# geometryxyz/mental-poker

Measured on AMD Instinct MI355X. Metric: shuffle proofs/sec (prove+verify), higher is better.
Workload: dtype u32 limbs (256-bit Montgomery: 9x29-bit lazy base field, 8x32 scalar field); 1 GPU; pairs: 52-card deck, m=2 n=26, stark curve, shuffle_and_remask + verify_shuffle; rccl_world=1, fixed_base_window_bits=21, unit_counted=prove+verify pairs, streams=1, aggregate_keys=1, transcript_lanes=1, prover_streams=1, pipeline_depth=0, validated_once=False, full=False

## Files before the change

### include/mpshuffle.h

```cpp
#ifndef MPSHUFFLE_H
#define MPSHUFFLE_H

#include <stddef.h>
#include <stdint.h>

#ifdef __cplusplus
extern "C" {
#endif

#define MP_CURVE_STARK 0
#define MP_CURVE_BN254 1
#define MP_CURVE_SECP256K1 2
#define MP_CURVE_BLS12_377 3

#define MP_OK 0
#define MP_ERR_BAD_ENCODING (-1)
#define MP_ERR_BAD_PERMUTATION (-2)
#define MP_ERR_BAD_ARGUMENT (-3)
#define MP_ERR_NO_DEVICE (-4)
#define MP_ERR_INTERNAL (-5)

typedef struct mp_ctx mp_ctx;
typedef struct mp_table mp_table;

int mp_ctx_create(int curve_id, int device, mp_ctx** out);
void mp_ctx_destroy(mp_ctx* ctx);
const char* mp_last_error(void);
const char* mp_check_name(int code);
size_t mp_proof_size(uint32_t m, uint32_t n);
size_t mp_params_size(uint32_t n);
size_t mp_point_size(int curve_id);
size_t mp_proof_size_curve(int curve_id, uint32_t m, uint32_t n);
size_t mp_params_size_curve(int curve_id, uint32_t n);

void* mp_host_alloc(size_t bytes);
void mp_host_free(void* p);
int mp_set_io_chunk(mp_table* t, size_t proofs);

int mp_setup(mp_ctx* ctx, uint32_t m, uint32_t n, const uint8_t seed[32], uint8_t* out_params);

int mp_table_create(mp_ctx* ctx, uint32_t m, uint32_t n, const uint8_t* params, const uint8_t* shared_key,
                    mp_table** out);
int mp_table_create_ex(mp_ctx* ctx, uint32_t m, uint32_t n, const uint8_t* params, const uint8_t* shared_key,
                       uint32_t fb_window_bits, mp_table** out);
uint32_t mp_table_window_bits(const mp_table* t);
void mp_table_destroy(mp_table* t);

int mp_shuffle_and_remask(mp_table* t, const uint8_t* deck, const uint8_t* masking_factors,
                          const uint32_t* permutation, const uint8_t prover_seed[32], uint8_t* out_deck,
                          uint8_t* out_proof);
int mp_verify_shuffle(mp_table* t, const uint8_t* deck, const uint8_t* shuffled_deck, const uint8_t* proof,
                      size_t proof_len);
int mp_shuffle_and_remask_keyed(mp_table* t, const uint8_t* shared_key, const uint8_t* deck, const uint8_t* masking_factors,
                                const uint32_t* permutation, const uint8_t prover_seed[32], uint8_t* out_deck, uint8_t* out_proof);
int mp_verify_shuffle_keyed(mp_table* t, const uint8_t* shared_key, const uint8_t* deck, const uint8_t* shuffled_deck,
                            const uint8_t* proof, size_t proof_len);
int mp_set_coalesce(mp_table* t, size_t max_batch, uint32_t max_wait_us);
int mp_coalesce_stats(const mp_table* t, uint64_t out[8]);

int mp_shuffle_and_remask_batch(mp_table* t, size_t B, const uint8_t* decks, const uint8_t* masking_factors,
                                const uint32_t* permutations, const uint8_t* prover_seeds, uint8_t* out_decks,
                                uint8_t* out_proofs, int32_t* status);
int mp_verify_shuffle_batch(mp_table* t, size_t B, const uint8_t* decks, const uint8_t* shuffled_decks,
                            const uint8_t* proofs, int32_t* status);

int mp_shuffle_and_remask_batch_dev(mp_table* t, size_t B, const void* d_decks, const void* d_masking_factors,
                                    const void* d_permutations, const void* d_prover_seeds, void* d_out_decks,
                                    void* d_out_proofs, void* d_status);
int mp_verify_shuffle_batch_dev(mp_table* t, size_t B, const void* d_decks, const void* d_shuffled_decks,
                                const void* d_proofs, void* d_status);
int mp_table_create_params(mp_ctx* ctx, uint32_t m, uint32_t n, const uint8_t* params, uint32_t fb_window_bits, mp_table** out);
int mp_shuffle_and_remask_batch_keys(mp_table* t, size_t B, const uint8_t* shared_keys, const uint8_t* decks,
                                     const uint8_t* masking_factors, const uint32_t* permutations, const uint8_t* prover_seeds,
                                     uint8_t* out_decks, uint8_t* out_proofs, int32_t* status);
int mp_verify_shuffle_batch_keys(mp_table* t, size_t B, const uint8_t* shared_keys, const uint8_t* decks,
                                 const uint8_t* shuffled_decks, const uint8_t* proofs, int32_t* status);
int mp_shuffle_and_remask_batch_keys_dev(mp_table* t, size_t B, const void* d_keys, const void* d_decks,
                                         const void* d_masking_factors, const void* d_permutations, const void* d_prover_seeds,
                                         void* d_out_decks, void* d_out_proofs, void* d_status);
int mp_verify_shuffle_batch_keys_dev(mp_table* t, size_t B, const void* d_keys, const void* d_decks, const void* d_shuffled_decks,
                                     const void* d_proofs, void* d_status);
typedef struct mp_keyset mp_keyset;
int mp_keyset_create(mp_table* t, size_t n_keys, const uint8_t* keys, mp_keyset** out);
void mp_keyset_destroy(mp_keyset* ks);
size_t mp_keyset_size(const mp_keyset* ks);
int mp_shuffle_and_remask_batch_keyset_dev(mp_table* t, const mp_keyset* ks, size_t B, const void* d_key_index, const void* d_decks,
                                           const void* d_masking_factors, const void* d_permutations, const void* d_prover_seeds,
                                           void* d_out_decks, void* d_out_proofs, void* d_status);
int mp_verify_shuffle_batch_keyset_dev(mp_table* t, const mp_keyset* ks, size_t B, const void* d_key_index, const void* d_decks,
                                       const void* d_shuffled_decks, const void* d_proofs, void* d_status);
int mp_verify_shuffle_chain(mp_table* t, size_t tables, uint32_t links, const uint8_t* shared_keys, const uint8_t* decks,
                            const uint8_t* proofs, int32_t* status);
int mp_verify_shuffle_chain_dev(mp_table* t, size_t tables, uint32_t links, const void* d_keys, const void* d_decks, const void* d_proofs,
                                void* d_status);
int mp_sync(mp_ctx* ctx);
int mp_reserve(mp_table* t, size_t B);
int mp_set_latency_batch(mp_table* t, size_t B);
int mp_set_work_split(mp_table* t, int split);
int mp_set_pipeline(mp_table* t, int depth);
int mp_set_plan_params(mp_table* t, int split, uint32_t fixed_terms, uint32_t var_terms, uint32_t table_group, uint32_t norm_chunk,
                       uint32_t window_lanes);
int mp_set_plan_thresholds(mp_table* t, size_t finest, size_t small, size_t latency, size_t medium, size_t wide);
int mp_set_merged_verify(mp_table* t, int on);
int mp_set_group_verify(mp_table* t, uint32_t points_per_group, size_t min_batch);
uint32_t mp_group_size(const mp_table* t, size_t B);
int mp_set_group_refine(mp_table* t, uint32_t points_per_subgroup, uint32_t min_subgroups);
uint64_t mp_reverified_count(const mp_table* t);
int mp_set_group_adapt(mp_table* t, int on);
int mp_set_bucket_min(mp_table* t, size_t terms);
int mp_set_bucket_bits(mp_table* t, uint32_t bits);
#define MP_VALIDATED_DECKS 1u
#define MP_VALIDATED_SHUFFLED 2u
#define MP_VALIDATED_PROOFS 4u
int mp_set_validated(mp_table* t, uint32_t what);
int mp_deck_validate_dev(mp_table* t, size_t decks, const void* d_wire_decks, void* d_status);
int mp_set_bucket_split(mp_table* t, uint32_t min_bits);
int mp_set_chain_max_links(mp_table* t, uint32_t links);
int mp_set_chain_group(mp_table* t, uint32_t tables_per_equation);
int mp_set_chain_slice(mp_table* t, size_t tables_per_pass);
uint32_t mp_chain_group_size(const mp_table* t, size_t tables, uint32_t links, int keyed);
size_t mp_chain_last_slice(const mp_table* t);
int mp_set_transcript_lanes(mp_table* t, uint32_t lanes);
int mp_set_group_lanes(mp_table* t, uint32_t lanes);
int mp_set_toom_cook(mp_table* t, int on);
int mp_set_subgroup_check(mp_table* t, int on);

int mp_remask_batch(mp_table* t, size_t count, const uint8_t* cards, const uint8_t* masking_factors, uint8_t* out);
int mp_msm(mp_table* t, size_t n_msm, size_t k, const uint8_t* scalars, const uint8_t* points, uint8_t* out);
int mp_commit_batch(mp_table* t, size_t count, size_t len, const uint8_t* values, const uint8_t* r, uint8_t* out);

int mp_sigma_prove_batch(mp_table* t, size_t B, uint32_t nbases, const uint8_t* bases, const uint8_t* publics,
                         const uint8_t* witness, const uint8_t* fs_init, const uint8_t* prover_seeds, uint8_t* out_proofs,
                         int32_t* status);
int mp_sigma_verify_batch(mp_table* t, size_t B, uint32_t nbases, const uint8_t* bases, const uint8_t* publics,
                          const uint8_t* proofs, const uint8_t* fs_init, int32_t* status);
int mp_blake2s(const uint8_t* in, size_t len, uint8_t out[32]);

size_t mp_serialized_point_size(int curve_id);
size_t mp_serialized_deck_size(int curve_id, size_t cards);
size_t mp_serialized_params_size(int curve_id, uint32_t n);
size_t mp_serialized_proof_size(int curve_id, uint32_t m, uint32_t n);
int mp_points_serialize(int curve_id, size_t count, const uint8_t* wire_points, uint8_t* out);
int mp_points_deserialize(int curve_id, size_t count, const uint8_t* data, uint8_t* out_wire_points);
int mp_deck_serialize(int curve_id, size_t cards, const uint8_t* wire_deck, uint8_t* out);
int mp_deck_deserialize(int curve_id, const uint8_t* data, size_t len, size_t max_cards, uint8_t* out_wire_deck, size_t* out_cards);
int mp_params_serialize(int curve_id, uint32_t m, uint32_t n, const uint8_t* raw_params, uint8_t* out);
int mp_params_deserialize(int curve_id, const uint8_t* data, size_t len, size_t max_n, uint32_t* m, uint32_t* n, uint8_t* out_raw_params);
int mp_proof_serialize(int curve_id, uint32_t m, uint32_t n, const uint8_t* proof_wire, uint8_t* out);
int mp_proof_deserialize(int curve_id, uint32_t m, uint32_t n, const uint8_t* data, size_t len, uint8_t* out_proof_wire);
int mp_points_deserialize_dev(mp_ctx* ctx, size_t count, const void* d_data, void* d_out_wire_points, void* d_status);
int mp_deck_deserialize_dev(mp_ctx* ctx, size_t decks, size_t cards, const void* d_data, void* d_out_wire_decks, void* d_status);

int mp_profile_enable(mp_ctx* ctx, int on);
int mp_profile_report(mp_ctx* ctx, char* buf, size_t buf_len);
int mp_work_census(mp_table* t, uint64_t* prove_terms, uint64_t* verify_terms, uint64_t* prove_point_ops,
                   uint64_t* verify_point_ops);

int mp_plan_stats(mp_table* t, uint64_t out[16]);

#ifdef __cplusplus
}
#endif
#endif
```

### mental-poker_amd/_native.py

```python
import ctypes
import os
import subprocess

HERE = os.path.dirname(os.path.abspath(__file__))
LIB_PATH = os.path.join(HERE, "libmpshuffle.so")
ROOT = os.path.dirname(HERE)

CURVE_IDS = {"stark": 0, "bn254": 1, "secp256k1": 2, "bls12_377": 3}
MP_ERR_BAD_ENCODING, MP_ERR_BAD_PERMUTATION, MP_ERR_BAD_ARGUMENT, MP_ERR_NO_DEVICE, MP_ERR_INTERNAL = -1, -2, -3, -4, -5

SYMBOLS = [
    "mp_ctx_create", "mp_ctx_destroy", "mp_last_error", "mp_check_name", "mp_proof_size", "mp_params_size",
    "mp_point_size", "mp_proof_size_curve", "mp_params_size_curve", "mp_set_merged_verify", "mp_set_subgroup_check", "mp_set_bucket_min", "mp_set_bucket_bits", "mp_set_bucket_split", "mp_set_validated", "mp_deck_validate_dev", "mp_set_chain_max_links", "mp_set_chain_group", "mp_set_chain_slice", "mp_chain_group_size", "mp_chain_last_slice", "mp_set_transcript_lanes", "mp_set_group_lanes", "mp_set_work_split", "mp_set_group_verify", "mp_group_size", "mp_set_group_refine", "mp_reverified_count", "mp_set_group_adapt", "mp_set_pipeline", "mp_set_plan_params", "mp_set_plan_thresholds", "mp_set_toom_cook", "mp_host_alloc", "mp_host_free", "mp_set_io_chunk", "mp_shuffle_and_remask_batch_keys", "mp_table_create_params",
    "mp_verify_shuffle_batch_keys", "mp_shuffle_and_remask_batch_keys_dev", "mp_verify_shuffle_batch_keys_dev",
    "mp_keyset_create", "mp_keyset_destroy", "mp_keyset_size", "mp_shuffle_and_remask_batch_keyset_dev", "mp_verify_shuffle_batch_keyset_dev",
    "mp_setup", "mp_table_create", "mp_table_create_ex", "mp_table_window_bits", "mp_table_destroy", "mp_shuffle_and_remask", "mp_verify_shuffle",
    "mp_shuffle_and_remask_keyed", "mp_verify_shuffle_keyed", "mp_set_coalesce", "mp_coalesce_stats",
    "mp_shuffle_and_remask_batch", "mp_verify_shuffle_batch", "mp_shuffle_and_remask_batch_dev",
    "mp_verify_shuffle_batch_dev", "mp_verify_shuffle_chain", "mp_verify_shuffle_chain_dev", "mp_sync", "mp_reserve", "mp_set_latency_batch", "mp_remask_batch", "mp_msm", "mp_commit_batch",
    "mp_profile_enable", "mp_profile_report", "mp_work_census", "mp_plan_stats", "mp_sigma_prove_batch",
    "mp_sigma_verify_batch", "mp_blake2s",
    "mp_serialized_point_size", "mp_serialized_deck_size", "mp_serialized_params_size", "mp_serialized_proof_size",
    "mp_points_serialize", "mp_points_deserialize", "mp_deck_serialize", "mp_deck_deserialize", "mp_params_serialize",
    "mp_params_deserialize", "mp_proof_serialize", "mp_proof_deserialize", "mp_points_deserialize_dev", "mp_deck_deserialize_dev",
]


class NativeError(RuntimeError):
    def __init__(self, code, text):
        super().__init__("mpshuffle error %d: %s" % (code, text))
        self.code = code


class NoDeviceError(NativeError):
    pass


SOURCES = ["capi.hip"] + [f % c for c in ("stark", "bn254", "secp256k1", "bls12_377") for f in ("curve_%s.hip", "curve_%s_msm.hip")]


def build(verbose=False):
    from concurrent.futures import ThreadPoolExecutor
    csrc = os.path.join(HERE, "csrc")
    objdir = os.path.join(csrc, "_obj")
    os.makedirs(objdir, exist_ok=True)
    headers = [os.path.join(csrc, f) for f in os.listdir(csrc) if f.endswith(".hpp")]
    headers.append(os.path.join(ROOT, "include", "mpshuffle.h"))
    hdr_time = max(os.path.getmtime(h) for h in headers)
    hipcc = os.environ.get("HIPCC", "/opt/rocm/bin/hipcc")
    flags = ["--offload-arch=gfx950", "-O3", "-std=c++17", "-fPIC", "-mllvm", "-amdgpu-sched-strategy=max-ilp",
             "-mllvm", "-pragma-unroll-threshold=1000000"]

    def compile_one(src):
        obj = os.path.join(objdir, src.replace(".hip", ".o"))
        spath = os.path.join(csrc, src)
        if os.path.exists(obj) and os.path.getmtime(obj) >= max(hdr_time, os.path.getmtime(spath)):
            return obj, False
        cmd = [hipcc] + flags + ["-c", spath, "-o", obj]
        if verbose:
            print(" ".join(cmd), flush=True)
        subprocess.check_call(cmd)
        return obj, True

    def compile_check():
        src = os.path.join(ROOT, "tools", "quadcheck", "quad_check.hip")
        exe = os.path.join(ROOT, "tools", "quadcheck", "quad_check")
        if not os.path.exists(src) or (os.path.exists(exe) and os.path.getmtime(exe) >= max(hdr_time, os.path.getmtime(src))):
            return
        cmd = [hipcc] + [f for f in flags if f != "-fPIC"] + ["-I", csrc, src, "-o", exe]
        if verbose:
            print(" ".join(cmd), flush=True)
        try:
            subprocess.check_call(cmd)
        except (subprocess.CalledProcessError, OSError) as e:
            print("warning: tools/quadcheck/quad_check did not build (%s); the library is unaffected" % e, flush=True)

    with ThreadPoolExecutor(max_workers=len(SOURCES) + 1) as ex:
        chk = ex.submit(compile_check)
        res = list(ex.map(compile_one, SOURCES))
        chk.result()
    objs = [r[0] for r in res]
    if any(r[1] for r in res) or not os.path.exists(LIB_PATH) or os.path.getmtime(LIB_PATH) < max(os.path.getmtime(o) for o in objs):
        cmd = [hipcc, "--offload-arch=gfx950", "-shared", "-fPIC", "-pthread", "-o", LIB_PATH] + objs
        if verbose:
            print(" ".join(cmd), flush=True)
        subprocess.check_call(cmd)
    mc = os.path.join(HERE, "mad_counts.json")
    gen = os.path.join(ROOT, "tools", "gen_mad_counts.py")
    if os.path.exists(gen) and (not os.path.exists(mc) or os.path.getmtime(mc) < max(hdr_time, os.path.getmtime(gen))):
        import importlib.util
        spec = importlib.util.spec_from_file_location("gen_mad_counts", gen)
        mod = importlib.util.module_from_spec(spec)
        spec.loader.exec_module(mod)
        mod.main([f for f in flags if f != "-fPIC"])
    return LIB_PATH


def bind(cdll):
    c = ctypes
    u8p, u32p, i32p = c.c_void_p, c.c_void_p, c.c_void_p
    cdll.mp_ctx_create.argtypes = [c.c_int, c.c_int, c.POINTER(c.c_void_p)]
    cdll.mp_ctx_destroy.argtypes = [c.c_void_p]
    cdll.mp_ctx_destroy.restype = None
    cdll.mp_last_error.restype = c.c_char_p
    cdll.mp_check_name.argtypes = [c.c_int]
    cdll.mp_check_name.restype = c.c_char_p
    cdll.mp_proof_size.argtypes = [c.c_uint32, c.c_uint32]
    cdll.mp_proof_size.restype = c.c_size_t
    cdll.mp_params_size.argtypes = [c.c_uint32]
    cdll.mp_params_size.restype = c.c_size_t
    cdll.mp_set_merged_verify.argtypes = [c.c_void_p, c.c_int]
    cdll.mp_set_subgroup_check.argtypes = [c.c_void_p, c.c_int]
    cdll.mp_set_bucket_min.argtypes = [c.c_void_p, c.c_size_t]
    cdll.mp_set_bucket_bits.argtypes = [c.c_void_p, c.c_uint32]
    cdll.mp_set_bucket_split.argtypes = [c.c_void_p, c.c_uint32]
    cdll.mp_set_validated.argtypes = [c.c_void_p, c.c_uint32]
    cdll.mp_deck_validate_dev.argtypes = [c.c_void_p, c.c_size_t, c.c_void_p, c.c_void_p]
    cdll.mp_set_toom_cook.argtypes = [c.c_void_p, c.c_int]
    cdll.mp_set_chain_max_links.argtypes = [c.c_void_p, c.c_uint32]
    cdll.mp_set_chain_group.argtypes = [c.c_void_p, c.c_uint32]
    cdll.mp_set_chain_slice.argtypes = [c.c_void_p, c.c_size_t]
    cdll.mp_chain_group_size.argtypes = [c.c_void_p, c.c_size_t, c.c_uint32, c.c_int]
    cdll.mp_chain_group_size.restype = c.c_uint32
    cdll.mp_chain_last_slice.argtypes = [c.c_void_p]
    cdll.mp_chain_last_slice.restype = c.c_size_t
    cdll.mp_set_transcript_lanes.argtypes = [c.c_void_p, c.c_uint32]
    cdll.mp_set_group_lanes.argtypes = [c.c_void_p, c.c_uint32]
    cdll.mp_set_work_split.argtypes = [c.c_void_p, c.c_int]
    cdll.mp_set_group_verify.argtypes = [c.c_void_p, c.c_uint32, c.c_size_t]
    cdll.mp_group_size.argtypes = [c.c_void_p, c.c_size_t]
    cdll.mp_group_size.restype = c.c_uint32
    cdll.mp_set_group_refine.argtypes = [c.c_void_p, c.c_uint32, c.c_uint32]
    cdll.mp_reverified_count.argtypes = [c.c_void_p]
    cdll.mp_set_group_adapt.argtypes = [c.c_void_p, c.c_int]
    cdll.mp_reverified_count.restype = c.c_uint64
    cdll.mp_set_pipeline.argtypes = [c.c_void_p, c.c_int]
    cdll.mp_set_plan_params.argtypes = [c.c_void_p, c.c_int] + [c.c_uint32] * 5
    cdll.mp_set_plan_thresholds.argtypes = [c.c_void_p] + [c.c_size_t] * 5
    cdll.mp_set_io_chunk.argtypes = [c.c_void_p, c.c_size_t]
    cdll.mp_host_alloc.argtypes = [c.c_size_t]
    cdll.mp_host_alloc.restype = c.c_void_p
    cdll.mp_host_free.argtypes = [c.c_void_p]
    cdll.mp_host_free.restype = None
    cdll.mp_point_size.argtypes = [c.c_int]
    cdll.mp_point_size.restype = c.c_size_t
    cdll.mp_proof_size_curve.argtypes = [c.c_int, c.c_uint32, c.c_uint32]
    cdll.mp_proof_size_curve.restype = c.c_size_t
    cdll.mp_params_size_curve.argtypes = [c.c_int, c.c_uint32]
    cdll.mp_params_size_curve.restype = c.c_size_t
    cdll.mp_setup.argtypes = [c.c_void_p, c.c_uint32, c.c_uint32, u8p, u8p]
    cdll.mp_table_create.argtypes = [c.c_void_p, c.c_uint32, c.c_uint32, u8p, u8p, c.POINTER(c.c_void_p)]
    cdll.mp_table_create_ex.argtypes = [c.c_void_p, c.c_uint32, c.c_uint32, u8p, u8p, c.c_uint32, c.POINTER(c.c_void_p)]
    cdll.mp_table_window_bits.argtypes = [c.c_void_p]
    cdll.mp_table_window_bits.restype = c.c_uint32
    cdll.mp_table_destroy.argtypes = [c.c_void_p]
    cdll.mp_table_destroy.restype = None
    cdll.mp_shuffle_and_remask.argtypes = [c.c_void_p, u8p, u8p, u32p, u8p, u8p, u8p]
    cdll.mp_verify_shuffle.argtypes = [c.c_void_p, u8p, u8p, u8p, c.c_size_t]
    cdll.mp_shuffle_and_remask_keyed.argtypes = [c.c_void_p, u8p, u8p, u8p, u32p, u8p, u8p, u8p]
    cdll.mp_verify_shuffle_keyed.argtypes = [c.c_void_p, u8p, u8p, u8p, u8p, c.c_size_t]
    cdll.mp_set_coalesce.argtypes = [c.c_void_p, c.c_size_t, c.c_uint32]
    cdll.mp_coalesce_stats.argtypes = [c.c_void_p, c.POINTER(c.c_uint64)]
    cdll.mp_shuffle_and_remask_batch.argtypes = [c.c_void_p, c.c_size_t, u8p, u8p, u32p, u8p, u8p, u8p, i32p]
    cdll.mp_verify_shuffle_batch.argtypes = [c.c_void_p, c.c_size_t, u8p, u8p, u8p, i32p]
    cdll.mp_shuffle_and_remask_batch_dev.argtypes = [c.c_void_p, c.c_size_t] + [c.c_void_p] * 7
    cdll.mp_verify_shuffle_batch_dev.argtypes = [c.c_void_p, c.c_size_t] + [c.c_void_p] * 4
    cdll.mp_table_create_params.argtypes = [c.c_void_p, c.c_uint32, c.c_uint32, u8p, c.c_uint32, c.POINTER(c.c_void_p)]
    cdll.mp_shuffle_and_remask_batch_keys.argtypes = [c.c_void_p, c.c_size_t, u8p, u8p, u8p, u32p, u8p, u8p, u8p, i32p]
    cdll.mp_verify_shuffle_batch_keys.argtypes = [c.c_void_p, c.c_size_t, u8p, u8p, u8p, u8p, i32p]
    cdll.mp_shuffle_and_remask_batch_keys_dev.argtypes = [c.c_void_p, c.c_size_t] + [c.c_void_p] * 8
    cdll.mp_verify_shuffle_batch_keys_dev.argtypes = [c.c_void_p, c.c_size_t] + [c.c_void_p] * 5
    cdll.mp_keyset_create.argtypes = [c.c_void_p, c.c_size_t, u8p, c.POINTER(c.c_void_p)]
    cdll.mp_keyset_destroy.argtypes = [c.c_void_p]
    cdll.mp_keyset_destroy.restype = None
    cdll.mp_keyset_size.argtypes = [c.c_void_p]
    cdll.mp_keyset_size.restype = c.c_size_t
    cdll.mp_shuffle_and_remask_batch_keyset_dev.argtypes = [c.c_void_p, c.c_void_p, c.c_size_t] + [c.c_void_p] * 8
    cdll.mp_verify_shuffle_batch_keyset_dev.argtypes = [c.c_void_p, c.c_void_p, c.c_size_t] + [c.c_void_p] * 5
    cdll.mp_verify_shuffle_chain.argtypes = [c.c_void_p, c.c_size_t, c.c_uint32, u8p, u8p, u8p, i32p]
    cdll.mp_verify_shuffle_chain_dev.argtypes = [c.c_void_p, c.c_size_t, c.c_uint32] + [c.c_void_p] * 4
    cdll.mp_sync.argtypes = [c.c_void_p]
    cdll.mp_reserve.argtypes = [c.c_void_p, c.c_size_t]
    cdll.mp_set_latency_batch.argtypes = [c.c_void_p, c.c_size_t]
    cdll.mp_remask_batch.argtypes = [c.c_void_p, c.c_size_t, u8p, u8p, u8p]
    cdll.mp_msm.argtypes = [c.c_void_p, c.c_size_t, c.c_size_t, u8p, u8p, u8p]
    cdll.mp_commit_batch.argtypes = [c.c_void_p, c.c_size_t, c.c_size_t, u8p, u8p, u8p]
    cdll.mp_profile_enable.argtypes = [c.c_void_p, c.c_int]
    cdll.mp_profile_report.argtypes = [c.c_void_p, c.c_char_p, c.c_size_t]
    cdll.mp_work_census.argtypes = [c.c_void_p] + [c.POINTER(c.c_uint64)] * 4
    cdll.mp_plan_stats.argtypes = [c.c_void_p, c.POINTER(c.c_uint64)]
    cdll.mp_sigma_prove_batch.argtypes = [c.c_void_p, c.c_size_t, c.c_uint32, u8p, u8p, u8p, u8p, u8p, u8p, i32p]
    cdll.mp_sigma_verify_batch.argtypes = [c.c_void_p, c.c_size_t, c.c_uint32, u8p, u8p, u8p, u8p, i32p]
    cdll.mp_blake2s.argtypes = [u8p, c.c_size_t, u8p]
    for fn, at in (("mp_serialized_point_size", [c.c_int]), ("mp_serialized_deck_size", [c.c_int, c.c_size_t]),
                   ("mp_serialized_params_size", [c.c_int, c.c_uint32]), ("mp_serialized_proof_size", [c.c_int, c.c_uint32, c.c_uint32])):
        getattr(cdll, fn).argtypes = at
        getattr(cdll, fn).restype = c.c_size_t
    cdll.mp_points_serialize.argtypes = [c.c_int, c.c_size_t, u8p, u8p]
    cdll.mp_points_deserialize.argtypes = [c.c_int, c.c_size_t, u8p, u8p]
    cdll.mp_deck_serialize.argtypes = [c.c_int, c.c_size_t, u8p, u8p]
    cdll.mp_deck_deserialize.argtypes = [c.c_int, u8p, c.c_size_t, c.c_size_t, u8p, c.POINTER(c.c_size_t)]
    cdll.mp_params_serialize.argtypes = [c.c_int, c.c_uint32, c.c_uint32, u8p, u8p]
    cdll.mp_params_deserialize.argtypes = [c.c_int, u8p, c.c_size_t, c.c_size_t, c.POINTER(c.c_uint32), c.POINTER(c.c_uint32), u8p]
    cdll.mp_points_deserialize_dev.argtypes = [c.c_void_p, c.c_size_t, c.c_void_p, c.c_void_p, c.c_void_p]
    cdll.mp_deck_deserialize_dev.argtypes = [c.c_void_p, c.c_size_t, c.c_size_t, c.c_void_p, c.c_void_p, c.c_void_p]
    cdll.mp_proof_serialize.argtypes = [c.c_int, c.c_uint32, c.c_uint32, u8p, u8p]
    cdll.mp_proof_deserialize.argtypes = [c.c_int, c.c_uint32, c.c_uint32, u8p, c.c_size_t, u8p]
    return cdll


_LIB = None


def load():
    global _LIB
    if _LIB is None:
        if not os.path.exists(LIB_PATH):
            raise ImportError("libmpshuffle.so is not built (run `python -c 'import __graft_entry__ as g; g.build()'`); "
# ... 31 lines not shown

    def points_deserialize(self, data):
        k = len(data) // self.cb
        if k * self.cb != len(data):
            raise NativeError(MP_ERR_BAD_ENCODING, "whole compressed points expected")
        out = (ctypes.c_uint8 * max(k * self.pb, 1))()
        self._chk(self.lib.mp_points_deserialize(self.cid, k, _in(data), out))
        return bytes(out)[:k * self.pb]

    def deck_serialize(self, wire):
        k = len(wire) // (2 * self.pb)
        if 2 * k * self.pb != len(wire):
            raise NativeError(MP_ERR_BAD_ARGUMENT, "whole cards expected")
        out = (ctypes.c_uint8 * self.lib.mp_serialized_deck_size(self.cid, k))()
        self._chk(self.lib.mp_deck_serialize(self.cid, k, _in(wire), out))
        return bytes(out)

    def deck_deserialize(self, data):
        cap = max(len(data) // (2 * self.cb), 1)
        out = (ctypes.c_uint8 * (cap * 2 * self.pb))()
        k = ctypes.c_size_t()
        self._chk(self.lib.mp_deck_deserialize(self.cid, _in(data), len(data), cap, out, ctypes.byref(k)))
        return bytes(out)[:k.value * 2 * self.pb]

    def params_serialize(self, m, n, raw):
        if len(raw) != self.pb * (n + 3):
            raise NativeError(MP_ERR_BAD_ARGUMENT, "parameters: wrong length")
        out = (ctypes.c_uint8 * self.lib.mp_serialized_params_size(self.cid, n))()
        self._chk(self.lib.mp_params_serialize(self.cid, m, n, _in(raw), out))
        return bytes(out)

    def params_deserialize(self, data):
        cap = max(len(data) // self.cb, 1)
        out = (ctypes.c_uint8 * (self.pb * (cap + 3)))()
        m, n = ctypes.c_uint32(), ctypes.c_uint32()
        self._chk(self.lib.mp_params_deserialize(self.cid, _in(data), len(data), cap, ctypes.byref(m), ctypes.byref(n), out))
        return m.value, n.value, bytes(out)[:self.pb * (n.value + 3)]

    def proof_serialize(self, m, n, wire):
        if len(wire) != self.lib.mp_proof_size_curve(self.cid, m, n):
            raise NativeError(MP_ERR_BAD_ARGUMENT, "proof: wrong length")
        out = (ctypes.c_uint8 * self.proof_serialized_size(m, n))()
        self._chk(self.lib.mp_proof_serialize(self.cid, m, n, _in(wire), out))
        return bytes(out)

    def proof_deserialize(self, m, n, data):
        out = (ctypes.c_uint8 * self.lib.mp_proof_size_curve(self.cid, m, n))()
        self._chk(self.lib.mp_proof_deserialize(self.cid, m, n, _in(data), len(data), out))
        return bytes(out)


class Engine:

    def __init__(self, curve="stark", device=0, lib=None):
        self.lib = lib if lib is not None else load()
        self.curve = curve
        h = ctypes.c_void_p()
        rc = self.lib.mp_ctx_create(CURVE_IDS[curve], device, ctypes.byref(h))
        if rc != 0:
            text = self.lib.mp_last_error().decode()
            raise (NoDeviceError if rc == MP_ERR_NO_DEVICE else NativeError)(rc, text)
        self.h = h
        self.point_bytes = self.lib.mp_point_size(CURVE_IDS[curve])

    def close(self):
        if getattr(self, "h", None):
            self.lib.mp_ctx_destroy(self.h)
            self.h = None

    def __del__(self):
        try:
            self.close()
        except Exception:
            pass

    def _chk(self, rc):
        if rc < 0:
            raise NativeError(rc, self.lib.mp_last_error().decode())
        return rc

    def check_name(self, code):
        return self.lib.mp_check_name(code).decode()

    def proof_size(self, m, n):
        return self.lib.mp_proof_size_curve(CURVE_IDS[self.curve], m, n)

    def blake2s(self, data):
        out = (ctypes.c_uint8 * 32)()
        self._chk(self.lib.mp_blake2s(_in(data), len(data), out))
        return bytes(out)

    def setup(self, m, n, seed):
        out = (ctypes.c_uint8 * self.lib.mp_params_size_curve(CURVE_IDS[self.curve], n))()
        self._chk(self.lib.mp_setup(self.h, m, n, _in(seed), out))
        return bytes(out)

    def table(self, m, n, params, shared_key, fb_bits=8):
        return Table(self, m, n, params, shared_key, fb_bits)

    def sync(self):
        self._chk(self.lib.mp_sync(self.h))

    def points_deserialize_dev(self, count, d_data, d_out_wire, d_status):
        self._chk(self.lib.mp_points_deserialize_dev(self.h, count, d_data, d_out_wire, d_status))

    def deck_deserialize_dev(self, decks, cards, d_data, d_out_wire_decks, d_status):
        self._chk(self.lib.mp_deck_deserialize_dev(self.h, decks, cards, d_data, d_out_wire_decks, d_status))

    def profile_enable(self, on=True):
        self._chk(self.lib.mp_profile_enable(self.h, 1 if on else 0))

    def profile_report(self):
        buf = ctypes.create_string_buffer(1 << 16)
        self._chk(self.lib.mp_profile_report(self.h, buf, len(buf)))
        out = {}
        self.last_profile_items = {}
        for line in buf.value.decode().splitlines():
            f = line.split()
            out[f[0]] = (int(f[1]), float(f[2]))
            if len(f) > 3:
                self.last_profile_items[f[0]] = int(f[3])
        return out


class KeySet:

    def __init__(self, table, keys):
        self.table, self.lib = table, table.lib
        if len(keys) == 0 or len(keys) % table.pb:
            raise ValueError("keys: expected a whole number of %d-byte points" % table.pb)
        self.size = len(keys) // table.pb
        h = ctypes.c_void_p()
        table.eng._chk(self.lib.mp_keyset_create(table.h, self.size, _in(keys), ctypes.byref(h)))
        self.h = h

    def close(self):
        if getattr(self, "h", None):
            self.lib.mp_keyset_destroy(self.h)
            self.h = None

    def __del__(self):
        try:
            self.close()
        except Exception:
            pass


class Table:

    def __init__(self, eng, m, n, params, shared_key, fb_bits=8):
        self.eng, self.lib, self.m, self.n, self.N = eng, eng.lib, m, n, m * n
        self.fb_bits = fb_bits
        self.params, self.shared_key = bytes(params), (bytes(shared_key) if shared_key is not None else None)
        self.pb = eng.point_bytes
        self.cb = 2 * eng.point_bytes
        if len(self.params) != self.pb * (n + 3) or (self.shared_key is not None and len(self.shared_key) != self.pb):
            raise NativeError(MP_ERR_BAD_ARGUMENT, "parameters / shared key have the wrong length")
        h = ctypes.c_void_p()
        if self.shared_key is None:
            eng._chk(self.lib.mp_table_create_params(eng.h, m, n, _in(self.params), fb_bits, ctypes.byref(h)))
        else:
            eng._chk(self.lib.mp_table_create_ex(eng.h, m, n, _in(self.params), _in(self.shared_key), fb_bits, ctypes.byref(h)))
        self.h = h
        self.fb_bits = self.lib.mp_table_window_bits(h)
        self.proof_bytes = eng.proof_size(m, n)

# ... 277 lines not shown
```

### mental-poker_amd/csrc/capi.hip

```cpp
#include <algorithm>
#include <cstring>

#include "engine_base.hpp"
#include "coalesce.hpp"

namespace mp {
std::string& last_error() {
  static thread_local std::string e;
  return e;
}
static inline size_t proof_size_bytes_(uint32_t m, uint32_t n) { return proof_size_bytes(m, n); }
}

using namespace mp;

#define MP_ENTER(CTX)                                          \
  std::lock_guard<std::recursive_mutex> mp_lock_((CTX)->mu);   \
  rt::set_device((CTX)->device)
#define MP_TRY try {
#define MP_CATCH                                                                     \
  }                                                                                  \
  catch (const std::invalid_argument& e) { return fail(MP_ERR_BAD_ENCODING, e.what()); } \
  catch (const std::exception& e) { return fail(MP_ERR_INTERNAL, e.what()); }

// ... 11 lines not shown
    case 0: return ser_scalars_ok_Stark(count, in);
    case 1: return ser_scalars_ok_Bn254(count, in);
    case 3: return ser_scalars_ok_Bls12_377(count, in);
    default: return ser_scalars_ok_Secp256k1(count, in);
  }
}
const int kCurveBits[4] = {252, 254, 256, 377};
struct Group {
  bool point;
  uint32_t count;
  bool vec;
  uint32_t vec_len;
};
std::vector<Group> proof_schema(uint32_t m, uint32_t n) {
  return {
      {true, m, true, m}, {true, m, true, m}, {true, 1, false, 0}, {true, m, true, m},
      {true, 1, false, 0}, {true, 1, false, 0}, {true, 2 * m + 1, true, 2 * m + 1},
      {false, n, true, n}, {false, n, true, n}, {false, 1, false, 0}, {false, 1, false, 0}, {false, 1, false, 0},
      {true, 1, false, 0}, {true, 1, false, 0}, {true, 1, false, 0},
      {false, n, true, n}, {false, n, true, n}, {false, 1, false, 0}, {false, 1, false, 0},
      {true, 1, false, 0}, {true, 2 * m, true, 2 * m}, {true, 4 * m, true, 2 * m},
      {false, n, true, n}, {false, 1, false, 0}, {false, 1, false, 0}, {false, 1, false, 0}, {false, 1, false, 0}};
}
void put_u64(uint8_t* p, uint64_t v) { memcpy(p, &v, 8); }
uint64_t get_u64(const uint8_t* p) {
  uint64_t v;
  memcpy(&v, p, 8);
  return v;
}
bool curve_ok(int c) { return c >= 0 && c <= 3; }
struct NoPipeline {
  mp_table* t;
  int keep;
  explicit NoPipeline(mp_table* tt) : t(tt), keep(tt->pipeline) {
    if (keep) t->flush();
    t->pipeline = 0;
  }
  ~NoPipeline() { t->pipeline = keep; }
};
}

extern "C" {

const char* mp_last_error(void) { return mp::last_error().c_str(); }
const char* mp_check_name(int code) {
  switch (code) {
    case 0: return "Ok";
    case 1: return "Hadamard Product (5.1)";
    case 2: return "Zero Argument (5.2)";
    case 3: return "Single Value Product (5.3)";
    case 4: return "Multi-Exponentiation Argument (4)";
    case 5: return "Schnorr Identification";
    case 6: return "Chaum-Pedersen";
    case MP_ERR_BAD_ENCODING: return "IoError: bad encoding";
    case MP_ERR_BAD_PERMUTATION: return "IoError: not a permutation";
    case MP_ERR_BAD_ARGUMENT: return "IoError: bad argument";
    case MP_ERR_NO_DEVICE: return "IoError: no MI355X device";
    default: return "IoError: internal";
  }
}
size_t mp_proof_size(uint32_t m, uint32_t n) { return proof_size_bytes(m, n); }
size_t mp_params_size(uint32_t n) { return (size_t)(n + 3) * 64; }
size_t mp_point_size(int curve_id) { return curve_id == MP_CURVE_BLS12_377 ? 96 : 64; }
size_t mp_proof_size_curve(int curve_id, uint32_t m, uint32_t n) { return proof_size_bytes(m, n, (uint32_t)mp_point_size(curve_id)); }
size_t mp_params_size_curve(int curve_id, uint32_t n) { return (size_t)(n + 3) * mp_point_size(curve_id); }

int mp_ctx_create(int curve_id, int device, mp_ctx** out) {
  if (!out) return fail(MP_ERR_BAD_ARGUMENT, "null out pointer");
  if (curve_id < 0 || curve_id > 3) return fail(MP_ERR_BAD_ARGUMENT, "unknown curve id");
  MP_TRY
  int ndev = rt::device_count();
  if (ndev <= 0 || device < 0 || device >= ndev)
    return fail(MP_ERR_NO_DEVICE, "no HIP device: libmpshuffle has no CPU path (runtime " MP_RT_NAME ")");
  rt::set_device(device);
  mp_ctx* c = new mp_ctx();
  c->curve = curve_id;
  c->device = device;
  c->stream = rt::stream_create();
  c->vstream = rt::stream_create();
  c->side = rt::stream_create();
  c->vside = rt::stream_create();
  c->h2d = c->vstream;
  c->d2h = c->vside;
  c->ev_fork = rt::event_create();
  c->ev_shuf = rt::event_create();
  c->ev_tab = rt::event_create();
  c->ev_vfork = rt::event_create();
  c->ev_vshuf = rt::event_create();
  c->ev_vtab = rt::event_create();
  c->ev_vin = rt::event_create();
  *out = c;
  return MP_OK;
  MP_CATCH
}
static void ctx_release(mp_ctx* ctx) {
  for (rt::Stream st : {ctx->stream, ctx->side, ctx->vstream, ctx->vside})
    if (st) rt::stream_destroy(st);
  for (rt::Event e : {ctx->ev_fork, ctx->ev_shuf, ctx->ev_tab, ctx->ev_vfork, ctx->ev_vshuf, ctx->ev_vtab, ctx->ev_vin})
    if (e) rt::event_destroy(e);
  delete ctx;
}
void mp_ctx_destroy(mp_ctx* ctx) {
  if (!ctx) return;
  {
    std::lock_guard<std::recursive_mutex> lock(ctx->mu);
    if (!ctx->tables.empty()) {
      ctx->dying = true;
      return;
    }
  }
  ctx_release(ctx);
}
int mp_setup(mp_ctx* ctx, uint32_t m, uint32_t n, const uint8_t seed[32], uint8_t* out_params) {
  if (!ctx || !seed || !out_params || m < 2 || n < 2) return fail(MP_ERR_BAD_ARGUMENT, "mp_setup: bad argument");
  MP_TRY
  MP_ENTER(ctx);
  switch (ctx->curve) {
    case 0: return setup_Stark(ctx, m, n, seed, out_params);
    case 1: return setup_Bn254(ctx, m, n, seed, out_params);
    case 3: return setup_Bls12_377(ctx, m, n, seed, out_params);
    default: return setup_Secp256k1(ctx, m, n, seed, out_params);
  }
  MP_CATCH
}

static uint32_t auto_window_bits(int curve, uint32_t n) {
  size_t free_b = 0, total_b = 0;
  rt::mem_info(&free_b, &total_b);
  const uint32_t sbits[4] = {252, 254, 256, 253};
  const size_t pbytes = curve == MP_CURVE_BLS12_377 ? 96 : 64;
  for (uint32_t bits : {21u, 20u, 16u}) {
    if (bits == 21 && sbits[curve] > 252) continue;
    const double tbl = (double)(n + 5) * ((sbits[curve] + bits - 1) / bits) * (double)((1u << bits) - 1u) * (double)pbytes;
    if (tbl <= 0.30 * (double)free_b && 3.3 * tbl <= 0.85 * (double)free_b) return bits;
  }
  return 8;
}
int mp_table_create(mp_ctx* ctx, uint32_t m, uint32_t n, const uint8_t* params, const uint8_t* shared_key, mp_table** out) {
  return mp_table_create_ex(ctx, m, n, params, shared_key, 0, out);
}
int mp_table_create_ex(mp_ctx* ctx, uint32_t m, uint32_t n, const uint8_t* params, const uint8_t* shared_key,
                       uint32_t fb_window_bits, mp_table** out) {
  if (!ctx || !params || !shared_key || !out) return fail(MP_ERR_BAD_ARGUMENT, "mp_table_create: null pointer");
  if (m < 2 || n < 2 || (uint64_t)m * n > 4096) return fail(MP_ERR_BAD_ARGUMENT, "mp_table_create: need m >= 2, n >= 2, m*n <= 4096");
  MP_TRY
  MP_ENTER(ctx);
  const bool auto_bits = fb_window_bits == 0;
  if (auto_bits) fb_window_bits = auto_window_bits(ctx->curve, n);
  int rc = MP_OK;
  mp_table* t = nullptr;
  auto make = [&](uint32_t bits) {
    switch (ctx->curve) {
      case 0: return make_table_Stark(ctx, m, n, params, shared_key, bits, &rc);
      case 1: return make_table_Bn254(ctx, m, n, params, shared_key, bits, &rc);
      case 3: return make_table_Bls12_377(ctx, m, n, params, shared_key, bits, &rc);
      default: return make_table_Secp256k1(ctx, m, n, params, shared_key, bits, &rc);
    }
  };
  if (!auto_bits) {
    t = make(fb_window_bits);
  } else {
    for (;;) {
      try {
        t = make(fb_window_bits);
        break;
      } catch (const std::exception& e) {
// ... 1 lines not shown
        if (fb_window_bits <= 8 || (!strstr(e.what(), "hipMalloc") && !strstr(e.what(), "memory"))) throw;
        fb_window_bits = fb_window_bits > 20 ? 20 : (fb_window_bits > 16 ? 16 : 8);
      }
    }
  }
  if (rc != MP_OK) {
    delete t;
    return rc;
  }
  t->co = new mp_coalescer();
  ctx->tables.push_back(t);
  *out = t;
  return MP_OK;
  MP_CATCH
}
int mp_table_create_params(mp_ctx* ctx, uint32_t m, uint32_t n, const uint8_t* params, uint32_t fb_window_bits, mp_table** out) {
  int rc = mp_table_create_ex(ctx, m, n, params, params, fb_window_bits, out);
  if (rc == MP_OK) (*out)->keyless = true;
  return rc;
}
void mp_table_destroy(mp_table* t) {
  if (!t) return;
  try {
    MP_ENTER(t->ctx);
    t->flush();
  } catch (...) {
  }
  mp_ctx* ctx = t->ctx;
  bool last = false;
  {
    std::lock_guard<std::recursive_mutex> lock(ctx->mu);
    auto& reg = ctx->tables;
    reg.erase(std::remove(reg.begin(), reg.end(), t), reg.end());
    for (auto& st : t->io) {
      if (st.up) rt::event_destroy(st.up);
      if (st.done) rt::event_destroy(st.done);
      if (st.down) rt::event_destroy(st.down);
    }
    delete t->co;
    delete t;
    last = ctx->dying && reg.empty();
  }
  if (last) ctx_release(ctx);
}
void* mp_host_alloc(size_t bytes) {
  try {
    return rt::host_alloc(bytes);
  } catch (const std::exception& e) {
    fail(MP_ERR_INTERNAL, e.what());
    return nullptr;
  }
}
void mp_host_free(void* p) { rt::host_free(p); }

uint32_t mp_table_window_bits(const mp_table* t) {
  if (!t) return 0;
  std::lock_guard<std::recursive_mutex> mp_lock_(t->ctx->mu);
  return t->fb_bits;
}
int mp_set_latency_batch(mp_table* t, size_t B) {
  if (!t) return fail(MP_ERR_BAD_ARGUMENT, "mp_set_latency_batch: null table");
  std::lock_guard<std::recursive_mutex> mp_lock_(t->ctx->mu);
  t->set_latency_batch(B);
  return MP_OK;
}
int mp_set_io_chunk(mp_table* t, size_t proofs) {
  if (!t) return fail(MP_ERR_BAD_ARGUMENT, "mp_set_io_chunk: null table");
  std::lock_guard<std::recursive_mutex> mp_lock_(t->ctx->mu);
  t->io_chunk = proofs;
  return MP_OK;
}
int mp_set_merged_verify(mp_table* t, int on) {
  if (!t) return fail(MP_ERR_BAD_ARGUMENT, "mp_set_merged_verify: null table");
  std::lock_guard<std::recursive_mutex> mp_lock_(t->ctx->mu);
  t->set_merged_verify(on != 0);
  return MP_OK;
}
int mp_set_group_refine(mp_table* t, uint32_t points_per_subgroup, uint32_t min_subgroups) {
  if (!t) return fail(MP_ERR_BAD_ARGUMENT, "mp_set_group_refine: null table");
  if (points_per_subgroup > BUCKET_TERMS_MAX - 4096) return fail(MP_ERR_BAD_ARGUMENT, "mp_set_group_refine: at most 585 728 points per equation");
  std::lock_guard<std::recursive_mutex> mp_lock_(t->ctx->mu);
  t->set_group_refine(points_per_subgroup, min_subgroups);
  return MP_OK;
}
uint64_t mp_reverified_count(const mp_table* t) {
  if (!t) return 0;
  std::lock_guard<std::recursive_mutex> mp_lock_(t->ctx->mu);
  return t->reverified();
}
int mp_set_group_adapt(mp_table* t, int on) {
  if (!t) return fail(MP_ERR_BAD_ARGUMENT, "mp_set_group_adapt: null table");
  std::lock_guard<std::recursive_mutex> mp_lock_(t->ctx->mu);
  t->set_group_adapt(on != 0);
  return MP_OK;
}
int mp_set_bucket_min(mp_table* t, size_t terms) {
  if (!t) return fail(MP_ERR_BAD_ARGUMENT, "mp_set_bucket_min: null table");
  MP_TRY
  MP_ENTER(t->ctx);
  t->set_bucket_min((uint32_t)std::min<size_t>(terms, 0x7FFFFFFFu));
  return MP_OK;
  MP_CATCH
}
int mp_set_bucket_bits(mp_table* t, uint32_t bits) {
  if (!t) return fail(MP_ERR_BAD_ARGUMENT, "mp_set_bucket_bits: null table");
  if (bits != 0 && (bits < 8 || bits > 14)) return fail(MP_ERR_BAD_ARGUMENT, "mp_set_bucket_bits: 0 (by size) or 8 .. 14");
  MP_TRY
  MP_ENTER(t->ctx);
  t->set_bucket_bits(bits);
  return MP_OK;
  MP_CATCH
}
int mp_set_bucket_split(mp_table* t, uint32_t min_bits) {
  if (!t) return fail(MP_ERR_BAD_ARGUMENT, "mp_set_bucket_split: null table");
  if (min_bits < 10 || min_bits > 15) return fail(MP_ERR_BAD_ARGUMENT, "mp_set_bucket_split: 10 .. 15 (none)");
  MP_TRY
  MP_ENTER(t->ctx);
  t->flush();
  t->bucket_split_bits = min_bits;
  return MP_OK;
  MP_CATCH
}
int mp_set_validated(mp_table* t, uint32_t what) {
  if (!t) return fail(MP_ERR_BAD_ARGUMENT, "mp_set_validated: null table");
  if (what & ~(MP_VALIDATED_DECKS | MP_VALIDATED_SHUFFLED | MP_VALIDATED_PROOFS)) return fail(MP_ERR_BAD_ARGUMENT, "mp_set_validated: unknown flag");
  MP_TRY
  MP_ENTER(t->ctx);
  t->flush();
  t->validated = what;
  return MP_OK;
  MP_CATCH
}
int mp_deck_validate_dev(mp_table* t, size_t decks, const void* d_wire_decks, void* d_status) {
  if (!t || !decks || !d_wire_decks || !d_status || decks >= ((size_t)1 << 31)) return fail(MP_ERR_BAD_ARGUMENT, "mp_deck_validate_dev: bad argument");
  MP_TRY
  MP_ENTER(t->ctx);
  t->validate_decks_dev(decks, (const uint8_t*)d_wire_decks, (int32_t*)d_status);
  return MP_OK;
  MP_CATCH
}
int mp_set_chain_max_links(mp_table* t, uint32_t links) {
  if (!t) return fail(MP_ERR_BAD_ARGUMENT, "mp_set_chain_max_links: null table");
  std::lock_guard<std::recursive_mutex> mp_lock_(t->ctx->mu);
  t->chain_max_links = links;
  return MP_OK;
}
int mp_set_chain_slice(mp_table* t, size_t tables_per_pass) {
  if (!t) return fail(MP_ERR_BAD_ARGUMENT, "mp_set_chain_slice: null table");
  std::lock_guard<std::recursive_mutex> mp_lock_(t->ctx->mu);
  t->chain_slice = tables_per_pass;
  return MP_OK;
}
int mp_set_chain_group(mp_table* t, uint32_t tables_per_equation) {
  if (!t) return fail(MP_ERR_BAD_ARGUMENT, "mp_set_chain_group: null table");
  if (tables_per_equation > 4094) return fail(MP_ERR_BAD_ARGUMENT, "mp_set_chain_group: at most 4 094 tables per equation");
  std::lock_guard<std::recursive_mutex> mp_lock_(t->ctx->mu);
  t->chain_group = tables_per_equation;
  return MP_OK;
}
int mp_set_transcript_lanes(mp_table* t, uint32_t lanes) {
  if (!t) return fail(MP_ERR_BAD_ARGUMENT, "mp_set_transcript_lanes: null table");
  if (lanes != 0 && lanes != 1 && lanes != 4) return fail(MP_ERR_BAD_ARGUMENT, "mp_set_transcript_lanes: 0 (by batch size), 1 or 4");
  std::lock_guard<std::recursive_mutex> mp_lock_(t->ctx->mu);
  t->fs_lanes = lanes;
  return MP_OK;
}
// ... 795 lines not shown
```

### mental-poker_amd/csrc/curve.hpp

```cpp
#pragma once
#include "field.hpp"

namespace mp {

template <class C>
struct Aff {
  Fe<typename C::FqP> x, y;
};
template <class C>
struct Jac {
  Fe<typename C::FqP> X, Y, Z;
};

template <class C>
struct Cofactor {
  static constexpr bool ONE = C::ID != 3;
  static constexpr uint32_t H[4] = {0x00000000u, 0x00000000u, 0x30000000u, 0x170b5d44u};
};

template <class C>
MP_HD bool aff_is_inf(const Aff<C>& a) {
  return fe_is_zero(a.x) && fe_is_zero(a.y);
}
template <class C>
// ... 78 lines not shown
  if (aff_is_inf<C>(q)) return;
  if (fe_is_zero(p.Z)) {
    p.X = q.x;
    p.Y = q.y;
    p.Z = fe_one<F>();
    return;
  }
  const Fe<F> Z1Z1 = fe_sqr<F>(p.Z);
  const Fe<F> U2 = fe_mul<F>(q.x, Z1Z1);
  const Fe<F> S2 = fe_mul<F>(fe_mul<F>(q.y, p.Z), Z1Z1);
  const Fe<F> H = fe_sub<F>(U2, p.X);
  const Fe<F> Rr = fe_sub<F>(S2, p.Y);
  if (fe_is_zero(H)) {
    if (fe_is_zero(Rr))
      jac_dbl_ip<C>(p);
    else
      p.Z = fe_zero<F>();
    return;
  }
  const Fe<F> HH = fe_sqr<F>(H);
  const Fe<F> HHH = fe_mul<F>(H, HH);
  const Fe<F> V = fe_mul<F>(p.X, HH);
  const Fe<F> X3 = fe_sub<F>(fe_sub<F>(fe_sqr<F>(Rr), HHH), fe_dbl<F>(V));
  p.Y = fe_sub<F>(fe_mul<F>(Rr, fe_sub<F>(V, X3)), fe_mul<F>(p.Y, HHH));
  p.Z = fe_mul<F>(p.Z, H);
  p.X = X3;
}
template <class C>
MP_HD Jac<C> jac_madd(const Jac<C>& p, const Aff<C>& q) {
  Jac<C> r = p;
  jac_madd_ip<C>(r, q);
  return r;
}

template <class C>
MP_HD void jac_add_ip(Jac<C>& p, const Jac<C>& q) {
  typedef typename C::FqP F;
  if (fe_is_zero(q.Z)) return;
  if (fe_is_zero(p.Z)) {
    p = q;
    return;
  }
  const Fe<F> Z1Z1 = fe_sqr<F>(p.Z), Z2Z2 = fe_sqr<F>(q.Z);
  const Fe<F> U1 = fe_mul<F>(p.X, Z2Z2), U2 = fe_mul<F>(q.X, Z1Z1);
  const Fe<F> S1 = fe_mul<F>(fe_mul<F>(p.Y, q.Z), Z2Z2), S2 = fe_mul<F>(fe_mul<F>(q.Y, p.Z), Z1Z1);
  const Fe<F> H = fe_sub<F>(U2, U1);
  const Fe<F> Rr = fe_sub<F>(S2, S1);
  if (fe_is_zero(H)) {
    if (fe_is_zero(Rr))
      jac_dbl_ip<C>(p);
    else
      p.Z = fe_zero<F>();
    return;
  }
  const Fe<F> HH = fe_sqr<F>(H);
  const Fe<F> HHH = fe_mul<F>(H, HH);
  const Fe<F> V = fe_mul<F>(U1, HH);
  const Fe<F> X3 = fe_sub<F>(fe_sub<F>(fe_sqr<F>(Rr), HHH), fe_dbl<F>(V));
  p.Y = fe_sub<F>(fe_mul<F>(Rr, fe_sub<F>(V, X3)), fe_mul<F>(S1, HHH));
  p.Z = fe_mul<F>(fe_mul<F>(p.Z, q.Z), H);
  p.X = X3;
}
template <class C>
MP_HD Jac<C> jac_add(const Jac<C>& p, const Jac<C>& q) {
  Jac<C> r = p;
  jac_add_ip<C>(r, q);
  return r;
}

template <class C>
struct Xyzz {
  Fe<typename C::FqP> X, Y, ZZ, ZZZ;
};
template <class C>
MP_HD Xyzz<C> xyzz_inf() {
  Xyzz<C> p;
  p.X = fe_one<typename C::FqP>();
  p.Y = fe_one<typename C::FqP>();
  p.ZZ = fe_zero<typename C::FqP>();
  p.ZZZ = fe_zero<typename C::FqP>();
  return p;
}
template <class C>
MP_HD void xyzz_dbl_ip(Xyzz<C>& p) {
  typedef typename C::FqP F;
  if (fe_is_zero(p.ZZ)) return;
  if (fe_is_zero(p.Y)) {
    p.ZZ = fe_zero<F>();
    p.ZZZ = fe_zero<F>();
    return;
  }
  const Fe<F> U = fe_dbl<F>(p.Y);
  const Fe<F> V = fe_sqr<F>(U);
  const Fe<F> W = fe_mul<F>(U, V);
  const Fe<F> S = fe_mul<F>(p.X, V);
  const Fe<F> XX = fe_sqr<F>(p.X);
  const Fe<F> M = C::A == 1 ? fe_triple_add<F>(XX, fe_sqr<F>(p.ZZ)) : fe_add<F>(fe_dbl<F>(XX), XX);
  const Fe<F> X3 = fe_sub_dbl<F>(fe_sqr<F>(M), S);
  p.Y = fe_mulsub<F>(M, fe_sub_lazy<F>(S, X3), W, p.Y);
  p.X = X3;
  p.ZZ = fe_mul<F>(V, p.ZZ);
  p.ZZZ = fe_mul<F>(W, p.ZZZ);
}
template <class C, bool PROBE = false>
MP_HD void xyzz_madd_signed_ip(Xyzz<C>& p, const Aff<C>& q, bool neg) {
  typedef typename C::FqP F;
  if (aff_is_inf<C>(q)) return;
  if (fe_is_zero(p.ZZ)) {
    p.X = q.x;
    p.Y = neg ? fe_neg<F>(q.y) : q.y;
    p.ZZ = fe_one<F>();
    p.ZZZ = fe_one<F>();
    return;
  }
  Fe<F> qy = q.y;
  if constexpr (LazySub<F>::ON) {
    const Fe<F> ny = fe_neg_lazy<F>(q.y);
#pragma unroll
    for (int i = 0; i < 9; ++i) qy.v[i] = neg ? ny.v[i] : q.y.v[i];
  } else {
    if (neg) qy = fe_neg<F>(q.y);
  }
  const Fe<F> Pd = fe_sub_wide<F>(fe_mul<F>(q.x, p.ZZ), p.X);
  const Fe<F> Rr = fe_sub_wide<F>(fe_mul<F>(qy, p.ZZZ), p.Y);
  if (fe_is_zero(Pd)) {
    if (!PROBE && fe_is_zero(Rr)) {
      xyzz_dbl_ip<C>(p);
    } else {
      p.ZZ = fe_zero<F>();
      p.ZZZ = fe_zero<F>();
    }
    return;
  }
  const Fe<F> PP = fe_sqr<F>(Pd);
  const Fe<F> PPP = fe_mul<F>(Pd, PP);
  const Fe<F> Q = fe_mul<F>(p.X, PP);
  const Fe<F> X3 = fe_sub_sub_dbl<F>(fe_sqr<F>(Rr), PPP, Q);
  p.Y = fe_mulsub<F>(Rr, fe_sub_lazy<F>(Q, X3), p.Y, PPP);
  p.X = X3;
  p.ZZ = fe_mul<F>(p.ZZ, PP);
  p.ZZZ = fe_mul<F>(p.ZZZ, PPP);
}
template <class C, bool PROBE = false>
MP_HD void xyzz_madd_ip(Xyzz<C>& p, const Aff<C>& q) {
  xyzz_madd_signed_ip<C, PROBE>(p, q, false);
}
template <class C, bool PROBE = false>
MP_HD void xyzz_add_ip(Xyzz<C>& p, const Xyzz<C>& q) {
  typedef typename C::FqP F;
  if (fe_is_zero(q.ZZ)) return;
  if (fe_is_zero(p.ZZ)) {
    p = q;
    return;
  }
  const Fe<F> U1 = fe_mul<F>(p.X, q.ZZ), U2 = fe_mul<F>(q.X, p.ZZ);
  const Fe<F> S1 = fe_mul<F>(p.Y, q.ZZZ), S2 = fe_mul<F>(q.Y, p.ZZZ);
  const Fe<F> Pd = fe_sub<F>(U2, U1);
  const Fe<F> Rr = fe_sub<F>(S2, S1);
  if (fe_is_zero(Pd)) {
    if (!PROBE && fe_is_zero(Rr)) {
      xyzz_dbl_ip<C>(p);
    } else {
      p.ZZ = fe_zero<F>();
      p.ZZZ = fe_zero<F>();
    }
    return;
  }
  const Fe<F> PP = fe_sqr<F>(Pd);
  const Fe<F> PPP = fe_mul<F>(Pd, PP);
  const Fe<F> Q = fe_mul<F>(U1, PP);
  const Fe<F> X3 = fe_sub_sub_dbl<F>(fe_sqr<F>(Rr), PPP, Q);
  p.Y = fe_mulsub<F>(Rr, fe_sub_lazy<F>(Q, X3), S1, PPP);
  p.X = X3;
  p.ZZ = fe_mul<F>(fe_mul<F>(p.ZZ, q.ZZ), PP);
  p.ZZZ = fe_mul<F>(fe_mul<F>(p.ZZZ, q.ZZZ), PPP);
}
template <class C>
MP_HD Jac<C> xyzz_to_jac(const Xyzz<C>& p) {
  typedef typename C::FqP F;
  Jac<C> j;
  if (fe_is_zero(p.ZZ)) return jac_inf<C>();
  j.X = fe_mul<F>(p.X, p.ZZ);
  j.Y = fe_mul<F>(p.Y, p.ZZZ);
  j.Z = p.ZZ;
  return j;
}

template <class C>
MP_HD Aff<C> jac_to_aff_with_zinv(const Jac<C>& j, const Fe<typename C::FqP>& zinv) {
  typedef typename C::FqP F;
  Fe<F> zi2 = fe_sqr<F>(zinv);
  Aff<C> a;
  a.x = fe_mul<F>(j.X, zi2);
  a.y = fe_mul<F>(fe_mul<F>(j.Y, zi2), zinv);
  return a;
}

}
```

### mental-poker_amd/csrc/engine_base.hpp

```cpp
#pragma once
#include <algorithm>
#include <cstring>
#include <deque>
#include <map>
#include <memory>
#include <sstream>
#include <string>
#include <mutex>
#include <vector>

#include "../../include/mpshuffle.h"
#include "hash.hpp"
#include "layout.hpp"

namespace mp {

std::string& last_error();
inline int fail(int code, const std::string& msg) {
  last_error() = msg;
  return code;
}

template <class T>
struct DevBuf {
// ... 10 lines not shown
    p = (T*)rt::dmalloc(count * sizeof(T));
    n = count;
    if (zero) rt::dzero(p, count * sizeof(T), s);
  }
  void upload(const std::vector<T>& v, rt::Stream s) {
    alloc(v.size() ? v.size() : 1, s, false);
    if (!v.empty()) rt::h2d(p, v.data(), v.size() * sizeof(T), s);
  }
};

struct Profiler {
  bool on = false;
  struct Rec {
    const char* name;
    rt::Event a, b;
    uint64_t items;
  };
  std::vector<Rec> recs;
  std::vector<rt::Event> pool;
  rt::Event get() {
    if (!pool.empty()) {
      rt::Event e = pool.back();
      pool.pop_back();
      return e;
    }
    return rt::event_create();
  }
  void begin(const char* name, rt::Stream s, uint64_t items = 0) {
    if (!on) return;
    Rec r{name, get(), get(), items};
    rt::event_record(r.a, s);
    recs.push_back(r);
  }
  void end(rt::Stream s) {
    if (!on) return;
    rt::event_record(recs.back().b, s);
  }
  std::string report() {
    std::map<std::string, std::pair<long, double>> acc;
    std::map<std::string, uint64_t> items;
    std::vector<std::string> order;
    for (auto& r : recs) {
      float ms = rt::event_ms(r.a, r.b);
      if (!acc.count(r.name)) order.push_back(r.name);
      acc[r.name].first += 1;
      acc[r.name].second += ms;
      items[r.name] += r.items;
      pool.push_back(r.a);
      pool.push_back(r.b);
    }
    recs.clear();
    std::ostringstream os;
    for (auto& k : order) os << k << " " << acc[k].first << " " << acc[k].second << " " << items[k] << "\n";
    return os.str();
  }
  ~Profiler() {
    for (auto& r : recs) {
      rt::event_destroy(r.a);
      rt::event_destroy(r.b);
    }
    for (auto e : pool) rt::event_destroy(e);
  }
};

}

struct mp_ctx {
  std::recursive_mutex mu;
  int curve = 0;
  int device = 0;
  mp::rt::Stream stream{};
  mp::rt::Stream h2d{}, d2h{};
  mp::rt::Stream side{};
  mp::rt::Event ev_fork{}, ev_shuf{}, ev_tab{};
  mp::rt::Stream vstream{}, vside{};
  mp::rt::Event ev_vfork{}, ev_vshuf{}, ev_vtab{}, ev_vin{};
  std::vector<mp_table*> tables;
  bool dying = false;
  mp::DevBuf<uint32_t> sq_ghalf, sq_hh, sq_rr, sq_chain;
  uint32_t sq_geom[4] = {0, 0, 0, 0};
  uint32_t sq_exp[12] = {0};
  mp::Profiler prof;
  uint32_t bk_slots = 0;
};
namespace mp {
struct LaneSwap {
  mp_ctx* c;
  explicit LaneSwap(mp_ctx* ctx) : c(ctx) { swap(); }
  ~LaneSwap() { swap(); }
  LaneSwap(const LaneSwap&) = delete;
  LaneSwap& operator=(const LaneSwap&) = delete;
  void swap() {
    std::swap(c->stream, c->vstream);
    std::swap(c->side, c->vside);
    std::swap(c->ev_fork, c->ev_vfork);
    std::swap(c->ev_shuf, c->ev_vshuf);
    std::swap(c->ev_tab, c->ev_vtab);
  }
};
}

static const uint32_t FSQ_MAX_BATCH = 32768;
static const uint32_t PROVE_INIT_WAVE_MAX = 32768;
static const uint32_t OVERLAP_MAX_BATCH = 32768;
static const uint32_t SCAL3D_SPLIT_MAX_BATCH = 4096;
#define MP_WAVE_RUN(NAME, C, nwaves, lds_words, args)                             \
  do {                                                                            \
    ctx->prof.begin(#NAME, ctx->stream, (uint64_t)(nwaves));                      \
    MP_WAVE_LAUNCH(NAME, C, ctx->stream, (nwaves), (lds_words), (args));          \
    ctx->prof.end(ctx->stream);                                                   \
  } while (0)
#define MP_RUN(NAME, C, nx, ny, args)                      \
  do {                                                     \
    ctx->prof.begin(#NAME, ctx->stream, (uint64_t)(nx) * (ny)); \
    MP_LAUNCH(NAME, C, ctx->stream, (nx), (ny), (args));   \
    ctx->prof.end(ctx->stream);                            \
  } while (0)

struct mp_io_stage {
  mp::DevBuf<uint8_t> in0, in1, in2, in3, out0, out1, keys;
  mp::DevBuf<uint32_t> perm;
  mp::DevBuf<int32_t> status;
  mp::rt::Event up = nullptr, done = nullptr, down = nullptr;
  bool used = false;
};
struct mp_keyset {
  mp_table* owner = nullptr;
  size_t K = 0;
  mp::DevBuf<uint32_t> wire;
  mp::DevBuf<uint32_t> FB;
  uint32_t bits = 0, windows = 0, entries = 0;
};
struct mp_coalescer;
struct mp_table {
  mp_ctx* ctx = nullptr;
  mp_coalescer* co = nullptr;
  mp_io_stage io[2];
  size_t io_chunk = 0;
  uint32_t m = 0, n = 0, N = 0;
  uint32_t point_bytes = 64;
  uint32_t fb_bits = 8;
  bool keyless = false;
  uint32_t bucket_bits = 0;
  uint32_t validated = 0;
  uint32_t bucket_split_bits = 12;
  uint32_t chain_max_links = 0;
  size_t chain_slice = 0;
  uint32_t chain_group = 0;
  uint32_t fs_lanes = 0;
  uint32_t group_lanes = 0;
  int forced_split = -1;
  int pipeline = 0;
  virtual ~mp_table() {}
  virtual void flush() = 0;
  virtual void reserve(size_t B) = 0;
  virtual void set_latency_batch(size_t B) = 0;
  virtual void set_merged_verify(bool on) = 0;
  virtual void set_subgroup_check(bool on) = 0;
  virtual void set_bucket_min(uint32_t terms) = 0;
  virtual void set_bucket_bits(uint32_t bits) = 0;
  virtual void set_toom_cook(bool on) = 0;
  virtual void set_group_verify(uint32_t links, size_t min_batch) = 0;
  virtual uint32_t group_size_of(size_t B) const = 0;
  virtual void set_group_refine(uint32_t points, uint32_t min_groups) = 0;
  virtual void set_group_adapt(bool on) = 0;
  virtual uint64_t reverified() const = 0;
  virtual int set_plan_params(int plan, uint32_t fch, uint32_t vch, uint32_t grp, uint32_t nch, uint32_t vsp) = 0;
  virtual void set_plan_thresholds(size_t tiny, size_t small, size_t latency, size_t medium, size_t wide) = 0;
  virtual void prove_dev(size_t B, const uint8_t* decks, const uint8_t* rho, const uint32_t* perm, const uint8_t* seeds,
                         uint8_t* out_decks, uint8_t* out_proofs, int32_t* status, const uint8_t* keys = nullptr,
                         const mp_keyset* ks = nullptr, const uint32_t* kidx = nullptr) = 0;
  virtual void verify_dev(size_t B, const uint8_t* decks, const uint8_t* shuf, const uint8_t* proofs, int32_t* status,
                          const uint8_t* keys = nullptr, const mp_keyset* ks = nullptr, const uint32_t* kidx = nullptr) = 0;
  virtual int keyset_build(mp_keyset& ks, size_t K, const uint8_t* keys_host) = 0;
  virtual void verify_chain_dev(size_t T, uint32_t L, const uint8_t* decks, const uint8_t* proofs, int32_t* status,
                                const uint8_t* keys = nullptr) = 0;
  virtual size_t chain_lane_bytes(uint32_t L, bool keyed) = 0;
  virtual size_t chain_lanes_held() const = 0;
  virtual void validate_decks_dev(size_t count, const uint8_t* decks, int32_t* status) = 0;
  virtual uint32_t chain_group_size(size_t T, uint32_t L, bool keyed) const = 0;
  size_t chain_last_slice = 0;
  virtual void remask_host(size_t count, const uint8_t* cards, const uint8_t* rho, uint8_t* out) = 0;
  virtual void msm_host(size_t n_msm, size_t k, const uint8_t* scalars, const uint8_t* points, uint8_t* out) = 0;
  virtual void commit_host(size_t count, size_t len, const uint8_t* values, const uint8_t* r, uint8_t* out) = 0;
  virtual void sigma_host(bool prove, size_t B, uint32_t nb, const uint8_t* bases, const uint8_t* publics, const uint8_t* witness,
                          const uint8_t* fs_init, const uint8_t* seeds, uint8_t* proofs, int32_t* status) = 0;
  virtual void census(uint64_t* pt, uint64_t* vt, uint64_t* po, uint64_t* vo) = 0;
  virtual void plan_stats(uint64_t out[16]) = 0;
};


namespace mp {
#define MP_DECLARE_CURVE(NAME)                                                                                          \
  mp_table* make_table_##NAME(mp_ctx* ctx, uint32_t m, uint32_t n, const uint8_t* params, const uint8_t* pk,           \
                              uint32_t fb_bits, int* rc);                                                              \
  int setup_##NAME(mp_ctx* ctx, uint32_t m, uint32_t n, const uint8_t seed[32], uint8_t* out);                                   \
  long ser_points_##NAME(bool de, size_t count, const uint8_t* in, uint8_t* out);                                                \
  int decompress_dev_##NAME(mp_ctx* ctx, size_t groups, uint32_t per_group, uint32_t prefix, const uint8_t* d_in, uint8_t* d_out, \
                            int32_t* d_status);                                                                                   \
// ... 7 lines not shown
```

### mental-poker_amd/csrc/engine_core.hpp

```cpp
#pragma once
#include "engine_base.hpp"
#include "kernels_bucket.hpp"
#include "kernels_decompress.hpp"
#include "kernels_sigma.hpp"
#include "serialize_host.hpp"
#include "setup_host.hpp"

namespace mp {

static const uint32_t FCHUNK = 8;
static const uint32_t VCHUNK = 64;
static const uint32_t NORM_CHUNK = 64;
static const uint32_t BUCKET_MIN = 2048;
static const uint32_t BUCKET_MIN_SMALL_BATCH = 512;

struct PhaseDev {
  DevBuf<Term> recode, tables, fterms, vterms, cterms, cterms2, cterms0;
  DevBuf<Job> fjobs, vjobs, cjobs, cjobs2, cjobs0;
  DevBuf<BJob> bjobs;
  DevBuf<Term> bterms;
  DevBuf<BTermPos> bpos;
  DevBuf<Job> wcjobs;
  DevBuf<Term> wcterms;
  DevBuf<BJob> wjobs;
// ... 597 lines not shown
    if ((uint64_t)count * ph.n_bterms >= ((uint64_t)1 << 32) || (uint64_t)count * ph.n_b * bw + 8ull * bucket_slots() >= ((uint64_t)1 << 32)) throw std::runtime_error(too_large);
    BRecodeArgs ra{S, D, ph.bterms.p, ph.bpos.p, sstride, bw, ph.n_bterms, dstride, c};
    MP_RUN(k_bucket_recode, C, count * ph.n_bterms, 1, ra);
    if (c >= bucket_split_bits) {
      const uint32_t NBK = bk_buckets(c), XW = XyzzWords<C>::N, gmax = bk_chunks(ph.b_kpad_max), units = bk_units(c);
      if (gmax > BK_CHUNKS_MAX) throw std::runtime_error("bucket method: more than 589 824 terms in one multi-scalar multiplication with windows of 12 bits or more");
      const size_t per_item = ((size_t)ph.b_kpad_max + (size_t)NBK * XW) * 4 + (size_t)gmax * bk_offs_row(c) * 2, per_eq = per_item * ph.n_b * bw;
      if (!bk_pass_eqs || bk_pass_bytes != per_eq) {
        size_t free_b = 0, total_b = 0;
        rt::mem_info(&free_b, &total_b);
        const size_t have = (w.bk_sorted.n + w.bk_park.n) * 4 + w.bk_offs.n * 2;
        const size_t budget = total_b ? std::min<size_t>((size_t)12 << 30, (free_b + have) / 4) : (size_t)1 << 30;
        bk_pass_eqs = (uint32_t)std::max<size_t>(1, std::min<size_t>(budget / per_eq, 0x7FFFFFFFu));
        bk_pass_bytes = per_eq;
      }
      const uint32_t pass = std::min(count, std::max(bk_pass_eqs, 1u));
      const size_t items_max = (size_t)pass * ph.n_b * bw;
      if (items_max * units >= ((uint64_t)1 << 32)) throw std::runtime_error(too_large);
      w.bk_sorted.alloc(items_max * ph.b_kpad_max, s, false);
      w.bk_offs.alloc(items_max * gmax * bk_offs_row(c), s, false);
      w.bk_park.alloc(items_max * NBK * XW, s, false);
      w.bk_quarters.alloc(items_max * 8 * XW, s, false);
      for (uint32_t e0 = 0; e0 < count; e0 += pass) {
        const uint32_t ne = std::min(pass, count - e0), items = ne * ph.n_b * bw;
        const uint32_t acc_lds = bk_acc_lds_words(c, gmax, XW, G_::PW), wpb = rt::waves_per_block(acc_lds), wgs = (items * units + wpb - 1) / wpb;
        BSplitArgs sa{D, w.P.p, w.J.p, ph.bjobs.p, ph.bterms.p, w.Bpad, bw, ph.n_b, dstride, link_stride, c, e0, ne, tile, tile_K,
                      w.bk_sorted.p, w.bk_offs.p, w.bk_park.p, ph.b_kpad_max, gmax, units, wpb, wgs, w.bk_quarters.p};
        ctx->prof.begin("k_bucket_sort", s, (uint64_t)items * gmax);
        MP_BLOCK_LAUNCH(k_bucket_sort, C, s, items * gmax, bk_sort_lds_words(c), sa);
        ctx->prof.end(s);
        MP_WAVE_RUN(k_bucket_acc, C, (wgs + 7u) / 8u * 8u * wpb, acc_lds, sa);
        MP_WAVE_RUN(k_bucket_list, C, (wgs + 7u) / 8u * 8u * wpb, acc_lds, sa);
        MP_WAVE_RUN(k_bucket_reduce, C, items * 4u, 64u * XW, sa);
        MP_RUN(k_bucket_final, C, items, 1, sa);
      }
      BFoldArgs fa{w.J.p, ph.bjobs.p, w.Bpad, bw, 0u, c};
      if (quad_ops(count, ph.n_b)) {
        BFoldQuadArgs qa{fa, count, ph.n_b};
        MP_WAVE_RUN(k_bucket_fold_q, C, quad_waves(count, ph.n_b), 0, qa);
      } else {
        MP_RUN(k_bucket_fold, C, count, ph.n_b, fa);
      }
      return;
    }
    const uint32_t nitems = count * ph.n_b * bw, nslots = std::min(nitems, bucket_slots());
    w.ensure_bucket(bucket_slots(), ph.b_kpad_max, c, XyzzWords<C>::N, s);
    rt::dzero(w.bk_counter.p, 8 * 4, s);
    BucketArgs ba{D, w.P.p, w.J.p, ph.bjobs.p, ph.bterms.p, w.Bpad, bw, ph.n_b, dstride, link_stride, c, nitems, nslots, w.bk_counter.p,
                  count, bk_xcd_affine && count >= 8u ? 8u : 1u, tile, tile_K, bk_stage ? 1u : 0u,
                  w.bk_sorted.p, w.bk_park.p, ph.b_kpad_max, nullptr};
#ifdef MP_EXP_BK_TIMING
    w.bk_timing.alloc((size_t)bucket_slots() * 8, s);
    ba.timing = w.bk_timing.p;
#endif
    ctx->prof.begin("k_bucket_msm", s, nitems);
    MP_WAVE_LAUNCH(k_bucket_msm, C, s, nslots, bk_lds_words(c, XyzzWords<C>::N), ba);
    ctx->prof.end(s);
#ifdef MP_EXP_BK_TIMING
    {
      std::vector<unsigned long long> tm((size_t)nslots * 4);
      rt::d2h(tm.data(), w.bk_timing.p, tm.size() * 8, s);
      rt::stream_sync(s);
      double sum[4] = {0, 0, 0, 0};
      for (size_t i = 0; i < tm.size(); ++i) sum[i & 3] += (double)tm[i];
      fprintf(stderr, "k_bucket_msm items %u slots %u bits %u kpad %u: cycles/wave sort %.0f ranks %.0f additions %.0f reduction %.0f\n", nitems, nslots, c,
              ph.b_kpad_max, sum[0] / nslots, sum[1] / nslots, sum[2] / nslots, sum[3] / nslots);
    }
#endif
    BFoldArgs fa{w.J.p, ph.bjobs.p, w.Bpad, bw, 0u, c};
    if (quad_ops(count, ph.n_b)) {
      BFoldQuadArgs qa{fa, count, ph.n_b};
      MP_WAVE_RUN(k_bucket_fold_q, C, quad_waves(count, ph.n_b), 0, qa);
    } else {
      MP_RUN(k_bucket_fold, C, count, ph.n_b, fa);
    }
  }
  void run_msms(PhaseDev& ph, Workspace& w, uint32_t B) {
    if (ph.n_f) {
      FixedArgs a{w.S.p, w.J.p, FB.p, ph.fjobs.p, ph.fterms.p, w.Bpad, fbg, w.Bpad};
      if (quad_ops(B, ph.n_f)) {
        FixedQuadArgs qa{a, B, ph.n_f};
        MP_WAVE_RUN(k_fixed_msm_q, C, quad_waves(B, ph.n_f), 0, qa);
      } else {
        MP_RUN(k_fixed_msm, C, B, ph.n_f, a);
      }
    }
    if (ph.n_v) {
      VarArgs a{w.D.p, w.T.p, w.J.p, ph.vjobs.p, ph.vterms.p, w.Bpad, nwin, ph.vsplit};
      const uint32_t nvl = ph.n_v * ph.vsplit;
#ifdef MP_EXP_VAR_LDS
      ctx->prof.begin("k_var_msm", ctx->stream);
      hipLaunchKernelGGL((k_var_msm<C>), dim3((B + 255u) / 256u, nvl), dim3(256), MP_EXP_VAR_LDS, ctx->stream, a, (uint32_t)B);
      ctx->prof.end(ctx->stream);
#else
      if (quad_ops(B, nvl)) {
        VarQuadArgs qa{a, B, nvl};
        MP_WAVE_RUN(k_var_msm_q, C, quad_waves(B, nvl), 0, qa);
      } else {
        MP_RUN(k_var_msm, C, B, nvl, a);
      }
#endif
      if (ph.n_wc) {
        CombineArgs ca{w.J.p, w.P.p, ph.wcjobs.p, ph.wcterms.p, w.Bpad};
        run_combine(ca, B, ph.n_wc);
      }
      if (ph.n_w) {
        BFoldArgs fa{w.J.p, ph.wjobs.p, w.Bpad, 0u, nwin, 0u};
        if (quad_ops(B, ph.n_w)) {
          BFoldQuadArgs qa{fa, B, ph.n_w};
          ctx->prof.begin("k_wfold_q", ctx->stream);
          MP_WAVE_LAUNCH(k_bucket_fold_q, C, ctx->stream, quad_waves(B, ph.n_w), 0, qa);
          ctx->prof.end(ctx->stream);
        } else {
          ctx->prof.begin("k_wfold", ctx->stream);
          MP_LAUNCH(k_bucket_fold, C, ctx->stream, B, ph.n_w, fa);
          ctx->prof.end(ctx->stream);
        }
      }
    }
    if (ph.n_b) run_bucket(w, ph, w.S.p, w.Bpad, w.D16.p, (size_t)w.d8_bytes, B, 0u, "bucket recode: batch too large for one launch");
    if (ph.n_c0) {
      CombineArgs a{w.J.p, w.P.p, ph.cjobs0.p, ph.cterms0.p, w.Bpad};
      run_combine(a, B, ph.n_c0);
    }
    if (ph.n_c) {
      CombineArgs a{w.J.p, w.P.p, ph.cjobs.p, ph.cterms.p, w.Bpad};
      run_combine(a, B, ph.n_c);
    }
    if (ph.n_c2) {
      CombineArgs a{w.J.p, w.P.p, ph.cjobs2.p, ph.cterms2.p, w.Bpad};
      run_combine(a, B, ph.n_c2);
    }
  }
  void run_normalize(PhaseDev& ph, Workspace& w, uint32_t B, uint32_t norm_only, uint32_t norm_skip, uint32_t* scratch) {
    std::vector<std::pair<uint32_t, uint32_t>> ranges;
    for (auto& r : ph.normalize)
      if ((norm_only == NO_SLOT || r.first == norm_only) && r.first != norm_skip) ranges.push_back(r);
    for (size_t i = 0; i < ranges.size();) {
      const size_t nr = std::min<size_t>(NORM_MAX_RANGES, ranges.size() - i);
      size_t last_elem = 0;
      for (size_t k = 0; k < nr; ++k)
        last_elem = std::max(last_elem, ((size_t)ranges[i + k].first + ranges[i + k].second) * w.Bpad);
      if (nr == 1 || last_elem >= ((size_t)1 << 32)) {
        auto& r = ranges[i];
        normalize_flat(w.J.p + j_off<C>(r.first, w.Bpad, 0), w.P.p + p_off<C>(r.first, w.Bpad, 0), scratch, (size_t)r.second * w.Bpad);
        ++i;
        continue;
      }
      NormMultiArgs a{};
      a.J = w.J.p; a.P = w.P.p; a.scratch = scratch;
      a.nr = (uint32_t)nr; a.chunk = cur_norm_chunk;
      uint32_t threads = 0, selem = 0;
      for (size_t k = 0; k < nr; ++k) {
        auto& r = ranges[i + k];
        const uint32_t cnt = r.second * w.Bpad;
        a.first[k] = r.first * w.Bpad;
        a.count[k] = cnt;
        a.tstart[k] = threads;
        a.sstart[k] = selem;
        threads += (cnt + cur_norm_chunk - 1) / cur_norm_chunk;
        selem += cnt;
      }
      a.tstart[nr] = threads;
      MP_RUN(k_normalize_multi, C, threads, 1, a);
      i += nr;
    }
  }

  FsStatementArgs statement_args(Workspace& w, uint32_t p_deck, uint32_t p_shuf, uint32_t p_cA, uint32_t s_x, uint32_t p_pk = NO_SLOT) {
    FsStatementArgs a{};
    a.f = FsDev{w.stage.p, w.seed.p, w.Bpad};
    a.S = w.S.p;
    a.P = w.P.p;
    a.fbpts = fbpts.p;
    memcpy(a.init_seed, init_seed, 32);
    a.m = m; a.n = n; a.N = N;
    a.p_deck = p_deck; a.p_shuf = p_shuf; a.p_cA = p_cA; a.s_x = s_x;
    a.p_pk = p_pk;
    a.W = nullptr;
    a.w_deck = a.w_shuf = NO_SLOT;
    return a;
  }
// ... 50 lines not shown
    mp_ctx* c;
    bool joined = false;
    ~SideGuard() {
      if (!joined) {
        try {
          rt::stream_sync(c->side);
        } catch (...) {
        }
      }
    }
  };
  void prove_side_work(PlanSet& q, Workspace& w, uint32_t B, bool with_tables) {
    const ProveLay& l = q.pplan.lay;
    run_phase(q.pph[4], w, B);
    const ToomPlan& tk = q.pplan.toom;
    if (tk.E) {
      ToomPointsArgs ta{w.P.p, w.J.p, w.Bpad, m, n, l.shuf, tk.cv_first};
      MP_RUN(k_toom_points, C, B, 2 * n, ta);
      normalize_flat(w.J.p + j_off<C>(tk.cv_first, w.Bpad, 0), w.P.p + p_off<C>(tk.cv_first, w.Bpad, 0), w.NS.p,
                     (size_t)(tk.E - 2) * 2 * n * w.Bpad);
    }
    if (with_tables) run_phase(q.pph[1], w, B, PH_TABLES);
  }

  void prove_dev(size_t B_, const uint8_t* decks, const uint8_t* rho, const uint32_t* perm, const uint8_t* seeds,
                 uint8_t* out_decks, uint8_t* out_proofs, int32_t* status, const uint8_t* keys, const mp_keyset* kset,
                 const uint32_t* kidx) override {
    const uint32_t B = (uint32_t)B_;
    const bool keyed = keys != nullptr || kset != nullptr;
    reserve_for(B, keyed);
    Workspace& w = ws;
    PlanSet& q = pick(B, keyed);
    cur_table_group = q.table_group;
    cur_norm_chunk = q.norm_chunk;
    const ProveLay& l = q.pplan.lay;
    PhaseDev* pph = q.pph;
    rt::Stream s = ctx->stream;
    FixedBases fb{n};
    const bool overlap = overlap_max && B <= overlap_max;
    SideGuard side_guard{ctx, !overlap};
    rt::dzero(w.status.p, (size_t)w.Bpad * 4, s);
    {
      uint32_t* const ww = wire_words(w, B, 1);
      LoadPointsArgs a{decks, w.P.p, w.status.p, w.Bpad, 2 * N, l.deck, ww, 0};
      MP_RUN(k_load_points, C, B, 2 * N, a);
      LoadScalarsArgs sa{rho, w.S.p, w.status.p, w.Bpad, N, l.rho};
      MP_RUN(k_load_scalars, C, B, N, sa);
      ProveInitArgs ia{w.S.p, w.status.p, perm, seeds, q.draws.p, l, w.Bpad};
      if (!overlap) prove_init(ia, B);
      RemaskArgs ra{w.S.p, w.P.p, w.J.p, FB.p, perm, w.Bpad, N, l.rho, l.deck, l.shuf, fb.G(), fb.pk(), fbg,
                    0, w.D.p, w.T.p, key_d_first, key_t_first, nwin, nullptr, nullptr, FbGeom{8, 32, 255}, 0};
      if (!(validated & MP_VALIDATED_DECKS)) check_subgroup(w, B, l.deck, 2 * N);
      if (kset) {
        keys = gather_keys(B, kset, kidx, w.status.p);
        LoadPointsArgs ka{keys, w.P.p, w.status.p, w.Bpad, 1, l.pk};
        MP_RUN(k_load_points, C, B, 1, ka);
        ra.keyed = 2;
        ra.KFB = kset->FB.p;
        ra.kidx = kidx;
        ra.kg = FbGeom{kset->bits, kset->windows, kset->entries};
        ra.nkeys = (uint32_t)kset->K;
      } else if (keyed) {
        LoadPointsArgs ka{keys, w.P.p, w.status.p, w.Bpad, 1, l.pk};
        MP_RUN(k_load_points, C, B, 1, ka);
        check_subgroup(w, B, l.pk, 1);
        KeyWinArgs kw{w.P.p, w.J.p, w.Bpad, l.pk, l.kw, nwin};
        MP_RUN(k_key_windows, C, B, 1, kw);
        normalize_flat(w.J.p + j_off<C>(l.kw, w.Bpad, 0), w.P.p + p_off<C>(l.kw, w.Bpad, 0), w.NS.p, (size_t)nwin * w.Bpad);
        RecodeArgs rc{w.S.p, w.D.p, key_recode.p, w.Bpad, nwin};
        MP_RUN(k_recode, C, B, N, rc);
        TableArgs ta{w.P.p, w.T.p, w.NS.p, key_tables.p, w.Bpad, nwin, cur_table_group};
        MP_RUN(k_table, C, B, (nwin + cur_table_group - 1) / cur_table_group, ta);
        ra.keyed = 1;
      }
      if (overlap) {
        struct Restore {
          mp_ctx* c;
          rt::Stream keep;
          ~Restore() { c->stream = keep; }
        } restore{ctx, s};
        rt::event_record(ctx->ev_fork, s);
        ctx->stream = ctx->side;
        rt::stream_wait(ctx->side, ctx->ev_fork);
        MP_RUN(k_remask, C, B, 2 * N, ra);
        run_phase(pph[0], w, B, PH_NORM, l.shuf);
        rt::event_record(ctx->ev_shuf, ctx->side);
        prove_side_work(q, w, B, true);
        rt::event_record(ctx->ev_tab, ctx->side);
      } else {
        MP_RUN(k_remask, C, B, 2 * N, ra);
      }
      if (overlap) {
        prove_init(ia, B);
        run_phase(pph[0], w, B, PH_ALL, NO_SLOT, l.shuf, w.NS2.p);
        rt::stream_wait(s, ctx->ev_shuf);
      } else {
        run_phase(pph[0], w, B);
        prove_side_work(q, w, B, false);
      }
    }
    const ToomPlan& tk = q.pplan.toom;
    {
      FsStatementArgs a = statement_args(w, l.deck, l.shuf, l.cA, l.x, keyed ? l.pk : NO_SLOT);
      a.W = wire_words(w, B, 1);
      a.w_deck = 0;
      run_fs_round1(a, B);
    }
    ProveScalArgs sc{w.S.p, perm, l, w.Bpad, q.lin.p, q.lin_src.p, tk.E ? 0u : (uint32_t)q.pplan.lin.size()};
    MP_RUN(k_prove_scal1, C, B, N, sc);
    MP_RUN(k_prove_scal1b, C, B, n + sc.n_lin * n, sc);
    MP_RUN(k_prove_scal1c, C, B, 1, sc);
    if (tk.E) {
      LinCombArgs la{w.S.p, q.lin.p, q.lin_src.p, q.lin_coef.p, q.consts.p, w.Bpad, n};
      MP_RUN(k_lin_comb, C, B, (uint32_t)q.pplan.lin.size() * n, la);
      FillConstArgs fa{w.S.p, q.consts.p, w.Bpad, tk.w_first, tk.w_const_first};
      MP_RUN(k_fill_consts, C, B, tk.E * tk.E, fa);
    }
    if (keyed) {
      KeyTermsArgs ka{w.S.p, w.J.p, w.Bpad, l.metau, q.pplan.jkey, kset ? 2u : 1u, w.T.p, key_t_first, nwin,
                      kset ? kset->FB.p : nullptr, kidx, kset ? FbGeom{kset->bits, kset->windows, kset->entries} : FbGeom{8, 32, 255},
                      kset ? (uint32_t)kset->K : 0u};
      MP_RUN(k_key_terms, C, B, 2 * m, ka);
    }
    if (overlap) {
      rt::stream_wait(s, ctx->ev_tab);
      side_guard.joined = true;
      run_phase(pph[1], w, B, PH_ALL & ~PH_TABLES);
    } else {
      run_phase(pph[1], w, B);
    }
    run_phase(pph[5], w, B);
    const FsDev f{w.stage.p, w.seed.p, w.Bpad};
    {
      FsRoundArgs a{};
      a.f = f; a.S = w.S.p; a.P = w.P.p;
      a.step[0] = FsStep{l.cB, m, 0, 0, l.y, l.z};
      a.nsteps = 1;
      a.copy_from = NO_SLOT; a.copy_to = NO_SLOT;
      run_fs_round(a, B);
    }
    MP_RUN(k_prove_scal2, C, B, n + 1, sc);
    MP_RUN(k_prove_scal2b, C, B, n, sc);
    run_phase(pph[2], w, B);
    {
      FsRoundArgs a{};
      a.f = f; a.S = w.S.p; a.P = w.P.p;
      a.copy_from = l.cb; a.copy_to = l.hB + m - 1;
      a.step[0] = FsStep{l.cb, 1, 0, 0, NO_SLOT, NO_SLOT};
      a.step[1] = FsStep{l.hB, m, 0, 0, l.hx, l.hy};
      a.nsteps = 2;
      run_fs_round(a, B);
    }
    MP_RUN(k_prove_scal3, C, B, n + 1, sc);
    {
      ProveScalArgs sd = sc;
      sd.d_parts = B <= SCAL3D_SPLIT_MAX_BATCH ? scal3d_parts(m, n) : 0u;
      if (sd.d_parts >= 2) {
        MP_RUN(k_prove_scal3d_part, C, B, (2 * m + 1) * sd.d_parts, sd);
      } else {
        sd.d_parts = 0;
      }
      MP_RUN(k_prove_scal3d, C, B, 2 * m + 1, sd);
    }
    run_phase(pph[3], w, B);
    {
      FsRoundArgs a{};
      a.f = f; a.S = w.S.p; a.P = w.P.p;
      a.copy_from = NO_SLOT; a.copy_to = NO_SLOT;
      a.step[0] = FsStep{l.zcA0, 2 + 2 * m + 1, 0, 0, l.zx, NO_SLOT};
      a.step[1] = FsStep{l.svcd, 3, 0, 0, l.svx, NO_SLOT};
      a.step[2] = FsStep{l.mecA0, 1 + 6 * m, 0, 0, l.mx, NO_SLOT};
      a.nsteps = 3;
      run_fs_round(a, B);
// ... 413 lines not shown
          else if (j < L) var(ChainTerm{l.mvar + l.deck + i, j * G + g, 1, l.mvar + l.shuf + i, G}, l.deck + i, j * G + g);
          else var(ChainTerm{l.mvar + l.shuf + i, (L - 1) * G + g, 1, NO_SLOT, G}, l.shuf + i, (L - 1) * G + g);
        }
    for (uint32_t j = 0; j < L * G; ++j)
      for (uint32_t slot = l.cA; slot < l.pk; ++slot) var(ChainTerm{l.mvar + slot, j, 1, NO_SLOT, 1}, slot, j);
    if (keyed)
      for (uint32_t g = 0; g < G; ++g) var(ChainTerm{l.mvar + l.pk, g, L, NO_SLOT, G}, l.pk, g);
    chain.K = (uint32_t)chain.cterms.size();
    FixedBases fb{n};
    for (uint32_t f = 0; f < fb.count(); ++f) {
      if (keyed && f == fb.pk()) continue;
      for (uint32_t j0 = 0; j0 < L * G; j0 += 64u) {
        pb.fixed((uint32_t)chain.cterms.size(), f);
        chain.cterms.push_back(ChainTerm{l.mfix + f, j0, std::min(64u, L * G - j0), NO_SLOT, 1});
      }
    }
    chain.nfix = (uint32_t)chain.cterms.size() - chain.K;
    pb.end();
    chain.nJ = next_partial;
    chain.dev.upload(chain.ph, ctx->stream);
    chain.dterms.upload(chain.cterms, ctx->stream);
    chain.dtile_src.upload(chain.tile_src, ctx->stream);
  }
  size_t chain_lane_bytes(uint32_t, bool keyed) override {
    if (keyed) ensure_keyed();
    const VerifyLay& l = (keyed ? psk : ps)[0].vplan.lay;
    const size_t fwb = (size_t)G_::FW * 4, nJ = 4 + bk_windows(R::BITS, 8);
    return (size_t)l.nS * 32 + (size_t)l.nP * 2 * fwb + nJ * 3 * fwb + nwin + (size_t)VB_ENTRIES * 2 * fwb + nJ * fwb + (size_t)stage_words_needed() * 4 + 32 + 8 + 4 + 8;
  }
  size_t chain_lanes_held() const override { return cws.cap; }
  uint32_t chain_group_size(size_t T, uint32_t L, bool keyed) const override { return T < 0x7FFFFFFFu ? chain_group_of((uint32_t)T, L, keyed) : 1u; }
  void verify_chain_dev(size_t T_, uint32_t L, const uint8_t* decks, const uint8_t* proofs, int32_t* status, const uint8_t* keys) override {
    const uint32_t T = (uint32_t)T_, B = T * L;
    const bool keyed = keys != nullptr;
    const uint32_t G = chain_group_of(T, L, keyed), Tq = T / G, Lq = L * G, Tpad = (Tq + 63u) & ~63u;
    build_chain_plan(L, keyed, G);
    PlanSet& q = (keyed ? psk : ps)[0];
    const VerifyLay& l = q.vplan.lay;
    rt::Stream s = ctx->stream;
    Workspace& w = cws;
    w.fw = G_::FW;
    w.ensure(B, l.nS, l.nP, std::max(chain.nJ, 8u), 0, 0, nwin, stage_words_needed(), s, 0);
    const size_t deck_bytes = (size_t)2 * N * G_::PB;
    rt::dzero(w.status.p, (size_t)w.Bpad * 4, s);
    {
      LoadPointsArgs a{decks, w.P.p, w.status.p, w.Bpad, 2 * N, l.deck};
      MP_RUN(k_load_points, C, B, 2 * N, a);
      LoadPointsArgs b{decks + (size_t)T * deck_bytes, w.P.p, w.status.p, w.Bpad, 2 * N, l.shuf};
      MP_RUN(k_load_points, C, B, 2 * N, b);
      ProofIoArgs pa{const_cast<uint8_t*>(proofs), w.S.p, w.P.p, w.status.p, q.vwire.p, w.Bpad, (uint32_t)proof_size_bytes(m, n, G_::PB)};
      MP_RUN(k_load_proof, C, B, (uint32_t)q.vplan.wire.size(), pa);
      if (keyed) {
        LoadPointsArgs ka{keys, w.P.p, w.status.p, w.Bpad, 1, l.pk};
        MP_RUN(k_load_points, C, B, 1, ka);
      }
      check_verify_inputs(w, B, l, keyed);
    }
    {
      VerifyFsArgs a{};
      a.st = statement_args(w, l.deck, l.shuf, l.cA, l.x, keyed ? l.pk : NO_SLOT);
      a.l = l;
      a.merge = 1u;
      run_verify_fs(a, B);
      VerifyScalArgs sa{w.S.p, w.P.p, w.direct.p, l, q.vplan.cm, w.Bpad};
      MP_RUN(k_verify_scal, C, B, n + 2, sa);
      VerifyMergeArgs ma{w.S.p, q.mjobs.p, q.mpairs.p, w.Bpad};
      MP_RUN(k_verify_merge, C, B, (uint32_t)q.vplan.mjobs.size(), ma);
    }
    const uint32_t nterms = chain.K + chain.nfix;
    chain_cw.alloc((size_t)Lq * Tpad * 8, s, false);
    chain_cs.alloc((size_t)nterms * Tpad * 8, s);
    chain_d8.alloc((size_t)chain.dev.b_dig_bytes * Tpad, s);
    run_chain_weights(w, Tpad, Tq, Lq);
    ChainScalArgs ca{w.S.p, chain_cw.p, chain_cs.p, chain.dterms.p, w.Bpad, Tpad, Tq};
    MP_RUN(k_chain_scalars, C, Tq, nterms, ca);
    PhaseDev& ph = chain.dev;
    DevBuf<uint32_t>& gt = gtile[0];
    gt.alloc((size_t)Tq * chain.K * G_::PW, s, false);
    ChainTileArgs ta{w.P.p, gt.p, chain.dtile_src.p, w.Bpad, Tq, chain.K};
    if ((uint64_t)Tq * chain.K >= ((uint64_t)1 << 32)) throw std::runtime_error("chain verification: too many tables for one launch");
    MP_RUN(k_chain_tile, C, Tq * chain.K, 1, ta);
    run_bucket(w, ph, chain_cs.p, Tpad, chain_d8.p, (size_t)ph.b_dig_bytes, Tq, Tq, "chain verification: too many tables for one launch", gt.p, chain.K);
    FixedArgs fx{chain_cs.p, w.J.p, FB.p, ph.fjobs.p, ph.fterms.p, w.Bpad, fbg, Tpad};
    MP_RUN(k_fixed_msm, C, Tq, ph.n_f, fx);
    if (ph.n_c0) {
      CombineArgs cb0{w.J.p, w.P.p, ph.cjobs0.p, ph.cterms0.p, w.Bpad};
      MP_RUN(k_combine, C, Tq, ph.n_c0, cb0);
    }
    CombineArgs cb{w.J.p, w.P.p, ph.cjobs.p, ph.cterms.p, w.Bpad};
    MP_RUN(k_combine, C, Tq, ph.n_c, cb);
    gbad[0].alloc(Tq, s, false);
    ChainVerdictArgs va{w.J.p, w.direct.p, w.status.p, flag_word(false, s), gbad[0].p, w.Bpad, Tq, Lq, 0u, w.P.p, keyed ? l.pk : NO_SLOT, G, status, nullptr};
    run_chain_verdict(va);
    if (!read_flag(false)) return;
    std::vector<uint32_t> bad, idx;
    read_words(gbad[0].p, Tq, bad);
    group_members(bad.data(), Tq, Lq, idx);
    const VArgs cv{B, decks, decks + (size_t)T * deck_bytes, proofs, status, keys, nullptr, nullptr};
    verify_subset(cv, idx, 0, false, 0, false);
  }

#ifndef MP_EXP_BK_TILE
#define MP_EXP_BK_TILE 1
#endif
#ifndef MP_EXP_BK_XCD
#define MP_EXP_BK_XCD 1
#endif
#ifndef MP_EXP_BK_STAGE
#define MP_EXP_BK_STAGE 1
#endif
  static constexpr bool bk_tile = MP_EXP_BK_TILE != 0, bk_xcd_affine = MP_EXP_BK_XCD != 0, bk_stage = MP_EXP_BK_STAGE != 0;
  DevBuf<uint32_t> gtile[2];
  std::map<std::pair<uint32_t, bool>, std::unique_ptr<ChainPlan>> gplans;
  Workspace gws;
  uint32_t bucket_bits_of(uint32_t K) const { return bucket_bits ? bucket_bits : bk_bits_for(K); }
  static const uint32_t GROUP_POINTS_WAVE = 30464u, GROUP_POINTS_WG = 243712u, GROUP_WG_POINTS_MIN = G_::FW > 8 ? 40000u : 50000u;
  uint32_t group_points = G_::FW > 8 ? 0u : GROUP_POINTS_WAVE;
  uint32_t group_points_wg = GROUP_POINTS_WG;
  uint32_t group_min_batch = 6144;
  void set_group_verify(uint32_t points, size_t min_batch) override {
    group_points = std::min(points, points > 65535u ? GROUP_POINTS_WAVE : 65535u);
    group_points_wg = points > 65535u ? points : 0u;
    group_min_batch = (uint32_t)std::min<size_t>(min_batch, 0x7FFFFFFFu);
  }
  uint32_t group_size_of(size_t B) const override { return B < 0x7FFFFFFFu ? group_size((uint32_t)B, false) : 0; }
  uint32_t group_size(uint32_t B, bool keyed) const {
    const uint32_t per = 4 * N + 11 * m + 8 + (keyed ? 1u : 0u);
    if ((!group_points && !group_points_wg) || !merged_verify || (uint64_t)B * N < (uint64_t)group_min_batch * 52u) return 0;
    const uint32_t groups_min = std::max<uint32_t>(1u, (uint32_t)(((uint64_t)group_min_batch * 2u) / 13u));
    uint32_t want = std::min<uint32_t>((group_points + per / 2) / per, B / groups_min);
    const uint32_t want_wg = std::min<uint32_t>((group_points_wg + per / 2) / per, B / std::max<uint32_t>(1u, group_min_batch / 512u));
    if (group_points_wg && (uint64_t)want_wg * per >= GROUP_WG_POINTS_MIN && (uint64_t)B * N * 3u >= (uint64_t)group_min_batch * 52u * 8u)
      want = std::max(want, want_wg);
    if (want >= 4) want = std::max<uint32_t>(want >> adapt_shift, 4u);
    if (want < 2) return 0;
    for (uint32_t d = 0; d <= want; ++d)
      for (int sgn = 1; sgn >= -1; sgn -= 2) {
        const int64_t L = (int64_t)want + sgn * (int64_t)d;
        if (L < 2 || 2 * L < (int64_t)want || L > 2 * (int64_t)want || (uint64_t)L * per + n + 5 > BUCKET_TERMS_MAX || (!bk_tile && L > 1023)) continue;
        if (B % (uint32_t)L == 0) return (uint32_t)L;
      }
    return 0;
  }
  uint32_t adapt_shift = 0;
  bool group_adapt = true;
  void set_group_adapt(bool on) override {
    group_adapt = on;
    adapt_shift = 0;
  }
  void note_group_verdicts(uint32_t T, uint32_t failing, uint32_t L) {
    if (!group_adapt || T < 8) return;
    if (T < 64 && failing > 0 && failing < 4) return;
    if ((uint64_t)failing * 5 > T) {
      const uint32_t by = (uint64_t)failing * 20 >= (uint64_t)T * 19 && L >= 128 ? 3u : 1u;
      if (L >= 16) adapt_shift = std::min<uint32_t>(7u, adapt_shift + by);
    } else if ((uint64_t)failing * 25 < T && adapt_shift > 0) {
      adapt_shift -= failing == 0 && adapt_shift >= 2 ? 2u : 1u;
    }
  }
  ChainPlan& build_group_plan(uint32_t L, bool keyed) {
    const std::pair<uint32_t, bool> key(L, keyed);
    auto it = gplans.find(key);
    if (it != gplans.end()) return *it->second;
    if (gplans.size() >= 8) {
      rt::stream_sync(ctx->stream);
      if (ctx->vstream) rt::stream_sync(ctx->vstream);
      gplans.clear();
// ... 25 lines not shown
        pb.fixed((uint32_t)gplan.cterms.size(), f);
        gplan.cterms.push_back(ChainTerm{l.mfix + f, j0, std::min(64u, L - j0), NO_SLOT, 1});
      }
    }
    gplan.nfix = (uint32_t)gplan.cterms.size() - gplan.K;
    pb.end();
    gplan.nJ = next_partial;
    gplan.dev.upload(gplan.ph, ctx->stream);
    gplan.dterms.upload(gplan.cterms, ctx->stream);
    return gplan;
  }
  void verify_group_pass(const VArgs& v, uint32_t L, bool vlane, uint32_t* host_flag, uint32_t* gbad_out) {
    const uint32_t B = v.B, T = B / L, Tpad = (T + 63u) & ~63u;
    const bool keyed = v.keys != nullptr || v.kset != nullptr;
    const uint8_t* keys = v.keys;
    ChainPlan& gplan = build_group_plan(L, keyed);
    PlanSet& q = (keyed ? psk : ps)[0];
    const VerifyLay& l = q.vplan.lay;
    rt::Stream s = ctx->stream;
    Workspace& w = vlane ? gws : ws;
    w.fw = G_::FW;
    w.ensure(B, l.nS, l.nP, std::max(gplan.nJ, 8u), 0, 0, nwin, stage_words_needed(), s, 0);
    rt::dzero(w.status.p, (size_t)w.Bpad * 4, s);
    {
      LoadPointsArgs a{v.decks, w.P.p, w.status.p, w.Bpad, 2 * N, l.deck};
      MP_RUN(k_load_points, C, B, 2 * N, a);
      LoadPointsArgs b{v.shuf, w.P.p, w.status.p, w.Bpad, 2 * N, l.shuf};
      MP_RUN(k_load_points, C, B, 2 * N, b);
      ProofIoArgs pa{const_cast<uint8_t*>(v.proofs), w.S.p, w.P.p, w.status.p, q.vwire.p, w.Bpad, (uint32_t)proof_size_bytes(m, n, G_::PB)};
      MP_RUN(k_load_proof, C, B, (uint32_t)q.vplan.wire.size(), pa);
      if (v.kset) keys = gather_keys(B, v.kset, v.kidx, w.status.p, vlane);
      if (keyed) {
        LoadPointsArgs ka{keys, w.P.p, w.status.p, w.Bpad, 1, l.pk};
        MP_RUN(k_load_points, C, B, 1, ka);
      }
      check_verify_inputs(w, B, l, keyed);
    }
    {
      VerifyFsArgs a{};
      a.st = statement_args(w, l.deck, l.shuf, l.cA, l.x, keyed ? l.pk : NO_SLOT);
      a.l = l;
      a.merge = 1u;
      run_verify_fs(a, B);
    }
    const uint32_t nterms = gplan.K + gplan.nfix;
    chain_cw.alloc((size_t)L * Tpad * 8, s, false);
    chain_cs.alloc((size_t)nterms * Tpad * 8, s);
    chain_d8.alloc((size_t)gplan.dev.b_dig_bytes * Tpad, s);
    {
      SideGuard wguard{ctx, false};
      rt::event_record(ctx->ev_fork, s);
      rt::stream_wait(ctx->side, ctx->ev_fork);
      {
        struct Restore {
          mp_ctx* c;
          rt::Stream keep;
          ~Restore() { c->stream = keep; }
        } restore{ctx, s};
        ctx->stream = ctx->side;
        run_chain_weights(w, Tpad, T, L);
        rt::event_record(ctx->ev_tab, ctx->side);
      }
      VerifyScalArgs sa{w.S.p, w.P.p, w.direct.p, l, q.vplan.cm, w.Bpad};
      MP_RUN(k_verify_scal, C, B, n + 2, sa);
      VerifyMergeArgs ma{w.S.p, q.mjobs.p, q.mpairs.p, w.Bpad};
      MP_RUN(k_verify_merge, C, B, (uint32_t)q.vplan.mjobs.size(), ma);
      rt::stream_wait(s, ctx->ev_tab);
      wguard.joined = true;
    }
    ChainScalArgs ca{w.S.p, chain_cw.p, chain_cs.p, gplan.dterms.p, w.Bpad, Tpad, T};
    MP_RUN(k_chain_scalars, C, T, nterms, ca);
    PhaseDev& ph = gplan.dev;
    const uint32_t* tile = nullptr;
    if (bk_tile) {
      const uint32_t per = l.pk + (keyed ? 1u : 0u);
      DevBuf<uint32_t>& gt = gtile[vlane ? 1 : 0];
      gt.alloc((size_t)T * gplan.K * G_::PW, s, false);
      GroupTileArgs ta{w.P.p, gt.p, w.Bpad, T, per, gplan.K};
      MP_RUN(k_group_tile, C, B, per, ta);
      tile = gt.p;
    }
    run_bucket(w, ph, chain_cs.p, Tpad, chain_d8.p, (size_t)ph.b_dig_bytes, T, T, "group verification: too many groups for one launch", tile, gplan.K);
    FixedArgs fx{chain_cs.p, w.J.p, FB.p, ph.fjobs.p, ph.fterms.p, w.Bpad, fbg, Tpad};
    MP_RUN(k_fixed_msm, C, T, ph.n_f, fx);
    if (ph.n_c0) {
      CombineArgs cb0{w.J.p, w.P.p, ph.cjobs0.p, ph.cterms0.p, w.Bpad};
      MP_RUN(k_combine, C, T, ph.n_c0, cb0);
    }
    CombineArgs cb{w.J.p, w.P.p, ph.cjobs.p, ph.cterms.p, w.Bpad};
    MP_RUN(k_combine, C, T, ph.n_c, cb);
    uint32_t* fl = host_flag;
    if (!fl) fl = flag_word(vlane, s);
    ChainVerdictArgs va{w.J.p, w.direct.p, w.status.p, fl, gbad_out, w.Bpad, T, L, 0u, w.P.p, NO_SLOT, 1u, v.status, nullptr};
    run_chain_verdict(va);
  }

  struct Adhoc {
    Phase ph;
    PhaseDev dev;
    Workspace w;
  };
  void run_adhoc(Adhoc& ad, uint32_t B, uint32_t nS, uint32_t nP, uint32_t nJ) {
    ad.dev.upload(ad.ph, ctx->stream);
    ad.w.fw = G_::FW;
    ad.w.ensure(B, nS, nP, nJ, ad.ph.n_dslots, ad.ph.n_tslots, nwin, 4, ctx->stream, ad.ph.b_dig_bytes);
  }

  void remask_host(size_t count, const uint8_t* cards, const uint8_t* rho, uint8_t* out) override {
    rt::Stream s = ctx->stream;
    const uint32_t B = (uint32_t)count;
    Adhoc ad;
    run_adhoc(ad, B, 1, 4, 4);
    Workspace& w = ad.w;
    DevBuf<uint8_t> din, drho, dout;
    din.alloc(count * 2 * G_::PB, s, false); drho.alloc(count * 32, s, false); dout.alloc(count * 2 * G_::PB, s, false);
    rt::h2d(din.p, cards, count * 2 * G_::PB, s);
    rt::h2d(drho.p, rho, count * 32, s);
    rt::dzero(w.status.p, (size_t)w.Bpad * 4, s);
    FixedBases fb{n};
    LoadPointsArgs a{din.p, w.P.p, w.status.p, w.Bpad, 2, 0};
    MP_RUN(k_load_points, C, B, 2, a);
    LoadScalarsArgs sa{drho.p, w.S.p, w.status.p, w.Bpad, 1, 0};
    MP_RUN(k_load_scalars, C, B, 1, sa);
    RemaskArgs ra{w.S.p, w.P.p, w.J.p, FB.p, nullptr, w.Bpad, 1, 0, 0, 2, fb.G(), fb.pk(), fbg, 0, nullptr, nullptr, 0, 0, 0};
    MP_RUN(k_remask, C, B, 2, ra);
    normalize_flat(w.J.p + j_off<C>(2, w.Bpad, 0), w.P.p + p_off<C>(2, w.Bpad, 0), w.NS.p, (size_t)2 * w.Bpad);
    StorePointsArgs st{dout.p, w.P.p, w.Bpad, 2, 2};
    MP_RUN(k_store_points, C, B, 2, st);
    std::vector<int32_t> hs(B);
    rt::d2h(out, dout.p, count * 2 * G_::PB, s);
    rt::d2h(hs.data(), w.status.p, (size_t)B * 4, s);
    rt::stream_sync(s);
    for (auto v : hs)
      if (v < 0) throw std::invalid_argument("remask: bad encoding in input");
  }

  void msm_host(size_t n_msm, size_t k, const uint8_t* scalars, const uint8_t* points, uint8_t* out) override {
    rt::Stream s = ctx->stream;
    const uint32_t B = (uint32_t)n_msm, K = (uint32_t)k;
    Adhoc ad;
    uint32_t next_partial = K + 1;
    {
      const uint32_t abits = bucket_bits_of(K);
      PhaseBuilder pb(ad.ph, next_partial, FCHUNK, VCHUNK, bucket_min, bk_windows(R::BITS, abits), 1u, abits);
      pb.begin(K);
      for (uint32_t t = 0; t < K; ++t) pb.var(t, t);
      pb.end();
      pb.normalize(K, 1);
    }
    run_adhoc(ad, B, K, K + 1, next_partial);
    Workspace& w = ad.w;
    DevBuf<uint8_t> dsc, dpt, dout;
    dsc.alloc(n_msm * k * 32, s, false); dpt.alloc(n_msm * k * G_::PB, s, false); dout.alloc(n_msm * G_::PB, s, false);
    rt::h2d(dsc.p, scalars, n_msm * k * 32, s);
    rt::h2d(dpt.p, points, n_msm * k * G_::PB, s);
    rt::dzero(w.status.p, (size_t)w.Bpad * 4, s);
    LoadPointsArgs la{dpt.p, w.P.p, w.status.p, w.Bpad, K, 0};
    MP_RUN(k_load_points, C, B, K, la);
    LoadScalarsArgs sa{dsc.p, w.S.p, w.status.p, w.Bpad, K, 0};
    MP_RUN(k_load_scalars, C, B, K, sa);
    run_phase(ad.dev, w, B);
    StorePointsArgs so{dout.p, w.P.p, w.Bpad, 1, K};
    MP_RUN(k_store_points, C, B, 1, so);
    std::vector<int32_t> hs(B);
    rt::d2h(out, dout.p, n_msm * G_::PB, s);
    rt::d2h(hs.data(), w.status.p, (size_t)B * 4, s);
    rt::stream_sync(s);
    for (auto v : hs)
      if (v < 0) throw std::invalid_argument("msm: bad encoding in input");
  }

  void commit_host(size_t count, size_t len, const uint8_t* values, const uint8_t* r, uint8_t* out) override {
    rt::Stream s = ctx->stream;
    const uint32_t B = (uint32_t)count, L = (uint32_t)len;
    FixedBases fb{n};
    Adhoc ad;
    uint32_t next_partial = 1;
    {
      PhaseBuilder pb(ad.ph, next_partial, FCHUNK, VCHUNK);
      pb.begin(0);
      for (uint32_t t = 0; t < L; ++t) pb.fixed(t, fb.ck(t));
      pb.fixed(L, fb.H());
      pb.end();
      pb.normalize(0, 1);
    }
    run_adhoc(ad, B, L + 1, 1, next_partial);
    Workspace& w = ad.w;
    DevBuf<uint8_t> dv, dr, dout;
    dv.alloc(std::max<size_t>(count * len * 32, 4), s, false); dr.alloc(count * 32, s, false); dout.alloc(count * G_::PB, s, false);
    if (len) rt::h2d(dv.p, values, count * len * 32, s);
    rt::h2d(dr.p, r, count * 32, s);
    rt::dzero(w.status.p, (size_t)w.Bpad * 4, s);
    if (L) {
      LoadScalarsArgs sa{dv.p, w.S.p, w.status.p, w.Bpad, L, 0};
      MP_RUN(k_load_scalars, C, B, L, sa);
    }
    LoadScalarsArgs sr{dr.p, w.S.p, w.status.p, w.Bpad, 1, L};
    MP_RUN(k_load_scalars, C, B, 1, sr);
    run_phase(ad.dev, w, B);
    StorePointsArgs so{dout.p, w.P.p, w.Bpad, 1, 0};
    MP_RUN(k_store_points, C, B, 1, so);
    std::vector<int32_t> hs(B);
    rt::d2h(out, dout.p, count * G_::PB, s);
    rt::d2h(hs.data(), w.status.p, (size_t)B * 4, s);
    rt::stream_sync(s);
    for (auto v : hs)
      if (v < 0) throw std::invalid_argument("commit: bad encoding in input");
  }
// ... 243 lines not shown
```

### mental-poker_amd/csrc/kernels_msm.hpp

```cpp
#pragma once
#include "curve.hpp"
#include "layout.hpp"

namespace mp {

template <class C>
struct Geo {
  static constexpr int OCC4 = C::FqP::NW > 8 ? 2 : 4;
  static constexpr int OCC3 = C::FqP::NW > 8 ? 2 : 3;
#ifdef MP_OCC_VAR
  static constexpr int OCC_VAR = MP_OCC_VAR;
#else
  static constexpr int OCC_VAR = OCC4;
#endif
  static constexpr int OCC_TABLE = C::FqP::NW > 8 ? 2 : (C::FqP::L29 ? 4 : 3);
  static constexpr uint32_t FW = C::FqP::NW;
  static constexpr uint32_t PW = 2 * FW;
  static constexpr uint32_t JW = 3 * FW;
  static constexpr uint32_t FB = 4 * FW;
  static constexpr uint32_t PB = 8 * FW;
};
template <int N>
MP_HD void ld_words(const uint32_t* p, uint32_t* v) {
  static_assert(N % 4 == 0, "elements are whole 16-byte vectors");
  const uint4* q = reinterpret_cast<const uint4*>(p);
#pragma unroll
  for (int i = 0; i < N / 4; ++i) {
    const uint4 t = q[i];
    v[4 * i] = t.x; v[4 * i + 1] = t.y; v[4 * i + 2] = t.z; v[4 * i + 3] = t.w;
  }
}
template <int N>
MP_HD void st_words(uint32_t* p, const uint32_t* v) {
  uint4* q = reinterpret_cast<uint4*>(p);
#pragma unroll
  for (int i = 0; i < N / 4; ++i) q[i] = make_uint4(v[4 * i], v[4 * i + 1], v[4 * i + 2], v[4 * i + 3]);
}
template <class F>
MP_HD Fe<F> ld_fe(const uint32_t* p) {
  uint32_t w[F::NW];
  ld_words<F::NW>(p, w);
  return fe_unpack<F>(w);
}
template <class F>
MP_HD void st_fe(uint32_t* p, const Fe<F>& a) {
  uint32_t w[F::NW];
  fe_pack<F>(a, w);
  st_words<F::NW>(p, w);
}
template <class F>
MP_HD void st_fe_lazy(uint32_t* p, const Fe<F>& a) {
  if constexpr (F::L29 && !F::PM29) {
    uint32_t w[F::NW];
    pack29<F::NW, F::NL29>(a.v, w);
    st_words<F::NW>(p, w);
  } else {
    st_fe<F>(p, a);
  }
}
template <class C>
MP_HD void st_aff_lazy(uint32_t* p, const Aff<C>& a) {
  st_fe_lazy<typename C::FqP>(p, a.x);
  st_fe_lazy<typename C::FqP>(p + Geo<C>::FW, a.y);
}
template <class C>
MP_HD Aff<C> ld_aff(const uint32_t* p) {
  Aff<C> a;
  a.x = ld_fe<typename C::FqP>(p);
  a.y = ld_fe<typename C::FqP>(p + Geo<C>::FW);
  return a;
}
template <class C>
MP_HD void st_aff(uint32_t* p, const Aff<C>& a) {
  st_fe<typename C::FqP>(p, a.x);
  st_fe<typename C::FqP>(p + Geo<C>::FW, a.y);
}
template <class C>
MP_HD Jac<C> ld_jac(const uint32_t* p) {
  Jac<C> j;
  j.X = ld_fe<typename C::FqP>(p);
  j.Y = ld_fe<typename C::FqP>(p + Geo<C>::FW);
  j.Z = ld_fe<typename C::FqP>(p + 2 * Geo<C>::FW);
  return j;
}
template <class C>
MP_HD void st_jac(uint32_t* p, const Jac<C>& j) {
  st_fe<typename C::FqP>(p, j.X);
  st_fe<typename C::FqP>(p + Geo<C>::FW, j.Y);
  st_fe<typename C::FqP>(p + 2 * Geo<C>::FW, j.Z);
}

MP_HD size_t s_off(uint32_t slot, uint32_t Bpad, uint32_t b) { return ((size_t)slot * Bpad + b) * 8; }
template <class C>
MP_HD size_t f_off(uint32_t slot, uint32_t Bpad, uint32_t b) { return ((size_t)slot * Bpad + b) * Geo<C>::FW; }
template <class C>
MP_HD size_t p_off(uint32_t slot, uint32_t Bpad, uint32_t b) { return ((size_t)slot * Bpad + b) * Geo<C>::PW; }
template <class C>
MP_HD size_t j_off(uint32_t slot, uint32_t Bpad, uint32_t b) { return ((size_t)slot * Bpad + b) * Geo<C>::JW; }

struct FbGeom {
  uint32_t bits, windows, entries;
};
struct FixedArgs {
  const uint32_t* S;
  uint32_t* J;
  const uint32_t* FB;
  const Job* jobs;
  const Term* terms;
  uint32_t Bpad;
  FbGeom g;
  uint32_t Sbpad;
};
template <class C>
MP_HD const uint32_t* fb_entry(const uint32_t* FB, const FbGeom& g, uint32_t base, uint32_t w, uint32_t d) {
  return FB + (((size_t)base * g.windows + w) * g.entries + (d - 1)) * Geo<C>::PW;
}
MP_HD uint32_t fb_digit(const uint32_t k[8], const FbGeom& g, uint32_t w) {
  const uint32_t bit = w * g.bits, word = bit >> 5, off = bit & 31;
  uint32_t v = k[word] >> off;
  if (off + g.bits > 32 && word < 7) v |= k[word + 1] << (32 - off);
  return v & ((1u << g.bits) - 1u);
}
template <class C>
MP_HD void body_fixed_msm(const FixedArgs& a, uint32_t b, uint32_t y) {
  typedef typename C::FrP R;
  const Job job = a.jobs[y];
  Xyzz<C> acc = xyzz_inf<C>();
  for (uint32_t t = 0; t < job.count; ++t) {
    const Term term = a.terms[job.begin + t];
    uint32_t k[8];
    fe_to_canonical<R>(ld_fe<R>(a.S + s_off(term.s, a.Sbpad, b)), k);
#pragma unroll 1
    for (uint32_t w = 0; w < a.g.windows; ++w) {
      const uint32_t d = fb_digit(k, a.g, w);
      if (d) xyzz_madd_ip<C>(acc, ld_aff<C>(fb_entry<C>(a.FB, a.g, term.b, w, d)));
    }
  }
  st_jac<C>(a.J + j_off<C>(job.out, a.Bpad, b), xyzz_to_jac<C>(acc));
}
MP_KERNEL_OCC(k_fixed_msm, FixedArgs, body_fixed_msm, Geo<C>::OCC4)

struct RemaskArgs {
  const uint32_t* S;
  const uint32_t* P;
  uint32_t* J;
  const uint32_t* FB;
  const uint32_t* perm;
  uint32_t Bpad, N;
  uint32_t s_rho, p_deck, j_out;
  uint32_t base_G, base_pk;
  FbGeom g;
  uint32_t keyed;
  const int8_t* D;
  const uint32_t* T;
  uint32_t d_first, t_first, nwin;
  const uint32_t* KFB;
  const uint32_t* kidx;
  FbGeom kg;
  uint32_t nkeys;
};
template <class C>
MP_HD void body_remask(const RemaskArgs& a, uint32_t b, uint32_t y) {
  typedef typename C::FrP R;
  const uint32_t i = y >> 1, comp = y & 1;
  uint32_t src = a.perm ? a.perm[(size_t)b * a.N + i] : i;
  if (src >= a.N) src = 0;
  uint32_t k[8];
  fe_to_canonical<R>(ld_fe<R>(a.S + s_off(a.s_rho + i, a.Bpad, b)), k);
  const uint32_t base = comp ? a.base_pk : a.base_G;
  Xyzz<C> acc = xyzz_inf<C>();
  if (a.keyed == 2 && comp) {
    uint32_t key = a.kidx[b];
    if (key >= a.nkeys) key = 0;
#pragma unroll 1
    for (uint32_t w = 0; w < a.kg.windows; ++w) {
      const uint32_t d = fb_digit(k, a.kg, w);
      if (d) xyzz_madd_ip<C>(acc, ld_aff<C>(fb_entry<C>(a.KFB, a.kg, key, w, d)));
    }
    xyzz_madd_ip<C>(acc, ld_aff<C>(a.P + p_off<C>(a.p_deck + 2 * src + comp, a.Bpad, b)));
    st_jac<C>(a.J + j_off<C>(a.j_out + y, a.Bpad, b), xyzz_to_jac<C>(acc));
    return;
  }
  if (a.keyed && comp) {
#pragma unroll 1
    for (uint32_t w = 0; w < a.nwin; ++w) {
      const int d = a.D[((size_t)(a.d_first + i) * a.nwin + w) * a.Bpad + b];
      if (d != 0) {
        const uint32_t e = (uint32_t)(d < 0 ? -d : d) - 1;
        const Aff<C> q = ld_aff<C>(a.T + p_off<C>((a.t_first + w) * VB_ENTRIES + e, a.Bpad, b));
        xyzz_madd_signed_ip<C>(acc, q, d < 0);
      }
    }
    xyzz_madd_ip<C>(acc, ld_aff<C>(a.P + p_off<C>(a.p_deck + 2 * src + comp, a.Bpad, b)));
    st_jac<C>(a.J + j_off<C>(a.j_out + y, a.Bpad, b), xyzz_to_jac<C>(acc));
    return;
  }
#pragma unroll 1
  for (uint32_t w = 0; w < a.g.windows; ++w) {
    const uint32_t d = fb_digit(k, a.g, w);
    if (d) xyzz_madd_ip<C>(acc, ld_aff<C>(fb_entry<C>(a.FB, a.g, base, w, d)));
  }
  xyzz_madd_ip<C>(acc, ld_aff<C>(a.P + p_off<C>(a.p_deck + 2 * src + comp, a.Bpad, b)));
  st_jac<C>(a.J + j_off<C>(a.j_out + y, a.Bpad, b), xyzz_to_jac<C>(acc));
}
MP_KERNEL_OCC(k_remask, RemaskArgs, body_remask, Geo<C>::OCC4)

struct KeyTermsArgs {
  const uint32_t* S;
  uint32_t* J;
  uint32_t Bpad, s_first, j_first;
  uint32_t keyed;
  const uint32_t* T;
  uint32_t t_first, nwin;
  const uint32_t* KFB;
  const uint32_t* kidx;
  FbGeom kg;
  uint32_t nkeys;
};
template <class C>
MP_HD void body_key_terms(const KeyTermsArgs& a, uint32_t b, uint32_t y) {
  typedef typename C::FrP R;
  uint32_t k[8];
  fe_to_canonical<R>(ld_fe<R>(a.S + s_off(a.s_first + y, a.Bpad, b)), k);
  Xyzz<C> acc = xyzz_inf<C>();
  if (a.keyed == 2) {
    uint32_t key = a.kidx[b];
    if (key >= a.nkeys) key = 0;
#pragma unroll 1
    for (uint32_t w = 0; w < a.kg.windows; ++w) {
      const uint32_t d = fb_digit(k, a.kg, w);
      if (d) xyzz_madd_ip<C>(acc, ld_aff<C>(fb_entry<C>(a.KFB, a.kg, key, w, d)));
    }
  } else {
    uint32_t carry = 0;
#pragma unroll 1
    for (uint32_t w = 0; w < a.nwin; ++w) {
      const uint32_t bit = w * VB_WINDOW_BITS, word = bit >> 5, off = bit & 31;
      uint32_t v = word < 8 ? k[word] >> off : 0u;
      if (off + VB_WINDOW_BITS > 32 && word < 7) v |= k[word + 1] << (32 - off);
      v = (v & ((1u << VB_WINDOW_BITS) - 1u)) + carry;
      carry = v > (1u << (VB_WINDOW_BITS - 1)) ? 1u : 0u;
      const int d = carry ? (int)v - (1 << VB_WINDOW_BITS) : (int)v;
      if (d != 0) {
        const uint32_t e = (uint32_t)(d < 0 ? -d : d) - 1;
        xyzz_madd_signed_ip<C>(acc, ld_aff<C>(a.T + p_off<C>((a.t_first + w) * VB_ENTRIES + e, a.Bpad, b)), d < 0);
      }
    }
  }
  st_jac<C>(a.J + j_off<C>(a.j_first + y, a.Bpad, b), xyzz_to_jac<C>(acc));
}
MP_KERNEL_OCC(k_key_terms, KeyTermsArgs, body_key_terms, Geo<C>::OCC4)

struct GatherKeysArgs {
  const uint32_t* wire;
  const uint32_t* kidx;
  uint32_t* out;
  int32_t* status;
  uint32_t nkeys;
};
template <class C>
MP_HD void body_gather_keys(const GatherKeysArgs& a, uint32_t b, uint32_t y) {
  constexpr uint32_t W = Geo<C>::PB / 4;
  uint32_t key = a.kidx[b];
  if (key >= a.nkeys) {
    if (y == 0) a.status[b] = -3;
    key = 0;
  }
  a.out[(size_t)b * W + y] = a.wire[(size_t)key * W + y];
}
MP_KERNEL(k_gather_keys, GatherKeysArgs, body_gather_keys)

struct KeyWinArgs {
  const uint32_t* P;
  uint32_t* J;
  uint32_t Bpad, p_pk, j_first, nwin;
};
template <class C>
MP_HD void body_key_windows(const KeyWinArgs& a, uint32_t b, uint32_t y) {
  Jac<C> acc = jac_from_aff<C>(ld_aff<C>(a.P + p_off<C>(a.p_pk, a.Bpad, b)));
  st_jac<C>(a.J + j_off<C>(a.j_first, a.Bpad, b), acc);
#pragma unroll 1
  for (uint32_t w = 1; w < a.nwin; ++w) {
#pragma unroll 1
    for (int q = 0; q < VB_WINDOW_BITS; ++q) jac_dbl_ip<C>(acc);
    st_jac<C>(a.J + j_off<C>(a.j_first + w, a.Bpad, b), acc);
  }
}
MP_KERNEL(k_key_windows, KeyWinArgs, body_key_windows)
// ... 72 lines not shown
  typedef typename C::FqP F;
  const uint32_t g0 = y * a.group;
  const uint32_t g1 = g0 + a.group < a.n_tables ? g0 + a.group : a.n_tables;
  Fe<F> prod = fe_one<F>();
  for (uint32_t g = g0; g < g1; ++g) {
    const Term t = a.list[g];
    const Aff<C> p1 = ld_aff<C>(a.P + p_off<C>(t.s, a.Bpad, b));
    st_aff<C>(a.T + p_off<C>(t.b * VB_ENTRIES, a.Bpad, b), p1);
    table_emit<C>(a, b, t.b, 1, 2, prod, fe_dbl<F>(p1.y));
  }
  bool desc = true;
#pragma unroll 1
  for (uint32_t e0 = 1; e0 < (uint32_t)VB_ENTRIES; e0 *= 2, desc = !desc) {
    Fe<F> inv = fe_inv<F>(prod);
    prod = fe_one<F>();
    const bool emit = 2 * e0 < (uint32_t)VB_ENTRIES;
    const uint32_t e0n = 2 * e0;
    for (uint32_t gi = 0; gi < g1 - g0; ++gi) {
      const uint32_t g = desc ? g1 - 1 - gi : g0 + gi;
      const uint32_t ts = a.list[g].b;
      const uint32_t* tb = a.T + p_off<C>(ts * VB_ENTRIES, a.Bpad, b);
      const size_t estride = (size_t)a.Bpad * Geo<C>::PW;
      if (e0 == 1) {
        const Aff<C> lo = ld_aff<C>(tb);
        const Aff<C> o2 = table_step<C>(a, b, ts, 1, 2, inv, lo, lo, true);
        table_emit<C>(a, b, ts, e0n, 4, prod, fe_dbl<F>(o2.y));
        table_emit<C>(a, b, ts, e0n, 3, prod, fe_sub<F>(o2.x, lo.x));
        continue;
      }
      const uint32_t h = e0 / 2;
      if (desc) {
        Aff<C> lo = ld_aff<C>(tb + (size_t)(e0 - 1) * estride), hi = lo;
        Fe<F> prevx = lo.x;
#pragma unroll 1
        for (uint32_t t = 2 * e0; t > e0; --t) {
          const bool dbl = (t & 1u) == 0;
          if (!dbl) {
            hi = lo;
            lo = ld_aff<C>(tb + (size_t)((t - 1) / 2 - 1) * estride);
          }
          const Aff<C> out = table_step<C>(a, b, ts, e0, t, inv, lo, hi, dbl);
          if (emit) {
            if (t < 2 * e0) table_emit<C>(a, b, ts, e0n, 2 * t + 1, prod, fe_sub<F>(prevx, out.x));
            table_emit<C>(a, b, ts, e0n, 2 * t, prod, fe_dbl<F>(out.y));
            prevx = out.x;
          }
        }
        if (emit)
          table_emit<C>(a, b, ts, e0n, 2 * e0 + 1, prod, fe_sub<F>(prevx, ld_fe<F>(tb + (size_t)(e0 - 1) * estride)));
      } else {
        Aff<C> lo = ld_aff<C>(tb + (size_t)(h - 1) * estride), hi = lo;
        Fe<F> prevx = lo.x;
        if (emit) prevx = ld_fe<F>(tb + (size_t)(e0 - 1) * estride);
#pragma unroll 1
        for (uint32_t t = e0 + 1; t <= 2 * e0; ++t) {
          const bool dbl = (t & 1u) == 0;
          if (!dbl) {
            if (t != e0 + 1) lo = hi;
            hi = ld_aff<C>(tb + (size_t)((t + 1) / 2 - 1) * estride);
          } else {
            lo = hi;
          }
          const Aff<C> out = table_step<C>(a, b, ts, e0, t, inv, lo, hi, dbl);
          if (emit) {
            table_emit<C>(a, b, ts, e0n, 2 * t - 1, prod, fe_sub<F>(out.x, prevx));
            table_emit<C>(a, b, ts, e0n, 2 * t, prod, fe_dbl<F>(out.y));
            prevx = out.x;
          }
        }
      }
    }
  }
}
MP_KERNEL_OCC(k_table, TableArgs, body_table, Geo<C>::OCC_TABLE)

struct VarArgs {
  const int8_t* D;
  const uint32_t* T;
  uint32_t* J;
  const Job* jobs;
  const Term* terms;
  uint32_t Bpad, nwin;
  uint32_t split;
};
template <class C>
MP_HD void body_var_msm(const VarArgs& a, uint32_t b, uint32_t y) {
  const uint32_t jidx = a.split > 1 ? y / a.split : y, r = y - jidx * a.split;
  const Job job = a.jobs[jidx];
  const int w_top = a.split > 1 ? (int)vsplit_lo(r + 1, a.split, a.nwin) - 1 : (int)a.nwin - 1;
  const int w_low = a.split > 1 ? (int)vsplit_lo(r, a.split, a.nwin) : 0;
  Xyzz<C> acc = xyzz_inf<C>();
#pragma unroll 1
  for (int w = w_top; w >= w_low; --w) {
    if (w != w_top) {
#pragma unroll 1
      for (int q = 0; q < VB_WINDOW_BITS; ++q) xyzz_dbl_ip<C>(acc);
    }
#pragma unroll 1
    for (uint32_t t = 0; t < job.count; ++t) {
      const Term term = a.terms[job.begin + t];
      const int d = a.D[((size_t)term.s * a.nwin + w) * a.Bpad + b];
      if (d != 0) {
        const uint32_t e = (uint32_t)(d < 0 ? -d : d) - 1;
        const Aff<C> q = ld_aff<C>(a.T + p_off<C>(term.b * VB_ENTRIES + e, a.Bpad, b));
        xyzz_madd_signed_ip<C>(acc, q, d < 0);
      }
    }
  }
  st_jac<C>(a.J + j_off<C>(job.out + r, a.Bpad, b), xyzz_to_jac<C>(acc));
}
MP_KERNEL_OCC(k_var_msm, VarArgs, body_var_msm, Geo<C>::OCC_VAR)

struct CombineArgs {
  uint32_t* J;
  const uint32_t* P;
  const Job* jobs;
  const Term* terms;
  uint32_t Bpad;
};
template <class C>
MP_HD void body_combine(const CombineArgs& a, uint32_t b, uint32_t y) {
  const Job job = a.jobs[y];
  Jac<C> acc = jac_inf<C>();
  for (uint32_t t = 0; t < job.count; ++t) {
    const uint32_t s = a.terms[job.begin + t].s;
    if (s & AFF_FLAG) {
      Aff<C> q = ld_aff<C>(a.P + p_off<C>(s & SLOT_MASK, a.Bpad, b));
      if (s & NEG_FLAG) q = aff_neg<C>(q);
      jac_madd_ip<C>(acc, q);
    } else {
      Jac<C> q = ld_jac<C>(a.J + j_off<C>(s & SLOT_MASK, a.Bpad, b));
      if (s & NEG_FLAG) q.Y = fe_neg<typename C::FqP>(q.Y);
      jac_add_ip<C>(acc, q);
    }
  }
  st_jac<C>(a.J + j_off<C>(job.out, a.Bpad, b), acc);
}
MP_KERNEL_OCC(k_combine, CombineArgs, body_combine, Geo<C>::OCC4)

struct NormArgs {
  const uint32_t* src;
  uint32_t* dst;
  uint32_t* scratch;
  uint32_t count, nthreads, chunk;
};
template <class C>
MP_HD void body_normalize(const NormArgs& a, uint32_t x, uint32_t y) {
  typedef typename C::FqP F;
  Fe<F> prod = fe_one<F>();
  uint32_t nmine = 0;
  for (uint32_t i = 0; i < a.chunk; ++i) {
    const size_t e = (size_t)x + (size_t)i * a.nthreads;
    if (e >= a.count) break;
    st_fe<F>(a.scratch + e * Geo<C>::FW, prod);
    Fe<F> z = ld_fe<F>(a.src + e * Geo<C>::JW + 2 * Geo<C>::FW);
    if (!fe_is_zero(z)) prod = fe_mul<F>(prod, z);
    nmine = i + 1;
  }
  Fe<F> inv = fe_inv<F>(prod);
  for (uint32_t i = nmine; i-- > 0;) {
    const size_t e = (size_t)x + (size_t)i * a.nthreads;
    Jac<C> j = ld_jac<C>(a.src + e * Geo<C>::JW);
    Aff<C> out = aff_inf<C>();
    if (!fe_is_zero(j.Z)) {
      Fe<F> before = ld_fe<F>(a.scratch + e * Geo<C>::FW);
      Fe<F> zinv = fe_mul<F>(inv, before);
      inv = fe_mul<F>(inv, j.Z);
      out = jac_to_aff_with_zinv<C>(j, zinv);
    }
    st_aff<C>(a.dst + e * Geo<C>::PW, out);
  }
}
MP_KERNEL(k_normalize, NormArgs, body_normalize)
static const uint32_t NORM_MAX_RANGES = 4;
struct NormMultiArgs {
  const uint32_t* J;
  uint32_t* P;
  uint32_t* scratch;
  uint32_t nr, chunk;
  uint32_t first[NORM_MAX_RANGES];
  uint32_t count[NORM_MAX_RANGES];
  uint32_t tstart[NORM_MAX_RANGES + 1];
  uint32_t sstart[NORM_MAX_RANGES];
};
template <class C>
MP_HD void body_normalize_multi(const NormMultiArgs& a, uint32_t x, uint32_t y) {
  uint32_t r = 0;
  while (r + 1 < a.nr && x >= a.tstart[r + 1]) ++r;
  NormArgs n;
  n.src = a.J + (size_t)a.first[r] * Geo<C>::JW;
  n.dst = a.P + (size_t)a.first[r] * Geo<C>::PW;
  n.scratch = a.scratch + (size_t)a.sstart[r] * Geo<C>::FW;
  n.count = a.count[r];
  n.nthreads = a.tstart[r + 1] - a.tstart[r];
// ... 74 lines not shown
    for (int i = 62; i >= 0; --i) {
      jac_dbl_ip<C>(q2);
      if ((C::SEED >> i) & 1u) jac_add_ip<C>(q2, q1);
    }
    bool ok = !jac_is_inf<C>(q2);
    const Fe<F> zz = fe_sqr<F>(q2.Z);
    ok = ok && fe_is_zero(fe_sub<F>(fe_mul<F>(fe_mul<F>(fe_unpack<F>(C::BETA_MONT), p.x), zz), q2.X));
    ok = ok && fe_is_zero(fe_add<F>(fe_mul<F>(fe_mul<F>(p.y, zz), q2.Z), q2.Y));
    return ok;
  } else {
    Jac<C> acc = jac_from_aff<C>(p);
#pragma unroll 1
    for (int i = R::BITS - 2; i >= 0; --i) {
      jac_dbl_ip<C>(acc);
      if ((R::MOD[i >> 5] >> (i & 31)) & 1u) jac_madd_ip<C>(acc, p);
    }
    return jac_is_inf<C>(acc);
  }
}
template <class C>
MP_HD void body_subgroup_check(const SubgroupArgs& a, uint32_t b, uint32_t y) {
  const Aff<C> p = ld_aff<C>(a.P + p_off<C>(a.p_first + y, a.Bpad, b));
  if (aff_is_inf<C>(p)) return;
  if (!aff_in_subgroup_dev<C>(p)) a.status[b] = -1;
}
MP_KERNEL_OCC(k_subgroup_check, SubgroupArgs, body_subgroup_check, 2)

struct FbWinArgs {
  const uint32_t* bases;
  uint32_t* WJ;
  FbGeom g;
  uint32_t bits2;
};
template <class C>
MP_HD void body_fb_windows(const FbWinArgs& a, uint32_t x, uint32_t y) {
  Jac<C> acc = jac_from_aff<C>(ld_aff<C>(a.bases + (size_t)x * Geo<C>::PW));
  for (uint32_t w = 0; w < a.g.windows; ++w) {
    st_jac<C>(a.WJ + ((size_t)x * a.g.windows + w) * Geo<C>::JW, acc);
    for (uint32_t q = 0; q < ((w & 1u) ? a.bits2 : a.g.bits); ++q) jac_dbl_ip<C>(acc);
  }
}
MP_KERNEL(k_fb_windows, FbWinArgs, body_fb_windows)
struct FbFillArgs {
  const uint32_t* W;
  uint32_t* EJ;
  FbGeom g;
};
template <class C>
MP_HD void body_fb_fill(const FbFillArgs& a, uint32_t x, uint32_t y) {
  const Aff<C> w = ld_aff<C>(a.W + (size_t)x * Geo<C>::PW);
  Jac<C> acc = jac_from_aff<C>(w);
  uint32_t* out = a.EJ + (size_t)x * a.g.entries * Geo<C>::JW;
  st_jac<C>(out, acc);
  jac_dbl_ip<C>(acc);
  st_jac<C>(out + Geo<C>::JW, acc);
  for (uint32_t e = 2; e < a.g.entries; ++e) {
    jac_madd_ip<C>(acc, w);
    st_jac<C>(out + (size_t)e * Geo<C>::JW, acc);
  }
}
MP_KERNEL(k_fb_fill, FbFillArgs, body_fb_fill)

struct FbWidenArgs {
  const uint32_t* Th;
  uint32_t* EJ;
  FbGeom gh, g;
};
template <class C>
MP_HD void body_fb_widen(const FbWidenArgs& a, uint32_t x, uint32_t y) {
  const uint32_t d = x % a.g.entries + 1u;
  const uint32_t bw = x / a.g.entries;
  const uint32_t base = bw / a.g.windows, w = bw % a.g.windows;
  const uint32_t hi = d >> a.gh.bits, lo = d & a.gh.entries;
  const uint32_t* tlo = a.Th + ((size_t)base * a.gh.windows + 2 * w) * a.gh.entries * Geo<C>::PW;
  Jac<C> acc = jac_inf<C>();
  if (lo) acc = jac_from_aff<C>(ld_aff<C>(tlo + (size_t)(lo - 1) * Geo<C>::PW));
  if (hi && 2 * w + 1 < a.gh.windows) jac_madd_ip<C>(acc, ld_aff<C>(tlo + ((size_t)a.gh.entries + hi - 1) * Geo<C>::PW));
  st_jac<C>(a.EJ + (size_t)x * Geo<C>::JW, acc);
}
MP_KERNEL(k_fb_widen, FbWidenArgs, body_fb_widen)

#define MP_MSM_KERNELS(X, C) \
  MP_KERNEL_INST(X, k_fixed_msm, FixedArgs, C) \
  MP_KERNEL_INST(X, k_remask, RemaskArgs, C) \
  MP_KERNEL_INST(X, k_key_windows, KeyWinArgs, C) \
  MP_KERNEL_INST(X, k_key_terms, KeyTermsArgs, C) \
  MP_KERNEL_INST(X, k_gather_keys, GatherKeysArgs, C) \
  MP_KERNEL_INST(X, k_recode, RecodeArgs, C) \
  MP_KERNEL_INST(X, k_table, TableArgs, C) \
  MP_KERNEL_INST(X, k_var_msm, VarArgs, C) \
  MP_KERNEL_INST(X, k_combine, CombineArgs, C) \
  MP_KERNEL_INST(X, k_normalize, NormArgs, C) \
  MP_KERNEL_INST(X, k_normalize_multi, NormMultiArgs, C) \
  MP_KERNEL_INST(X, k_fb_windows, FbWinArgs, C) \
  MP_KERNEL_INST(X, k_fb_fill, FbFillArgs, C) \
  MP_KERNEL_INST(X, k_fb_widen, FbWidenArgs, C) \
  MP_KERNEL_INST(X, k_subgroup_check, SubgroupArgs, C) \
  MP_KERNEL_INST(X, k_toom_points, ToomPointsArgs, C)

}
```

### mental-poker_amd/csrc/layout.hpp

```cpp
#pragma once
#include <algorithm>
#include <cstdint>
#include <map>
#include <stdexcept>
#include <vector>

#include "rt.hpp"

namespace mp {

struct Job {
  uint32_t out;
  uint32_t begin;
  uint32_t count;
};
struct Term {
  uint32_t s;
  uint32_t b;
};
struct BJob {
  uint32_t out;
  uint32_t win_first;
  uint32_t begin;
  uint32_t count;
  uint32_t kpad;
  uint32_t dig_off;
};
struct BTermPos {
  uint32_t pos;
  uint32_t kpad;
};
static const uint32_t AFF_FLAG = 0x80000000u;
static const uint32_t NEG_FLAG = 0x40000000u;
static const uint32_t SLOT_MASK = 0x3FFFFFFFu;
static const uint32_t NO_SLOT = 0xFFFFFFFFu;

struct FixedBases {
  uint32_t n;
  MP_HD uint32_t ck(uint32_t j) const { return j; }
  MP_HD uint32_t H() const { return n; }
  MP_HD uint32_t G() const { return n + 1; }
  MP_HD uint32_t pk() const { return n + 2; }
  MP_HD uint32_t gen() const { return n + 3; }
  MP_HD uint32_t gsum() const { return n + 4; }
  MP_HD uint32_t count() const { return n + 5; }
};

static const int VB_WINDOW_BITS = 5;
static const int VB_ENTRIES = 16;
static const uint32_t KEY_WINDOWS = 52;
static inline int vb_windows(int scalar_bits) { return (scalar_bits + 1 + VB_WINDOW_BITS - 1) / VB_WINDOW_BITS; }
MP_HD uint32_t vsplit_lo(uint32_t r, uint32_t k, uint32_t nwin) { return r * nwin / k; }
static const uint32_t VSPLIT_MAX = 16;

struct Phase {
  std::vector<Term> recode;
  std::vector<Term> tables;
  std::vector<Job> fjobs, vjobs, cjobs, cjobs2;
  std::vector<Term> fterms, vterms, cterms, cterms2;
  std::vector<Job> cjobs0;
  std::vector<Term> cterms0;
  std::vector<std::pair<uint32_t, uint32_t>> normalize;
  uint32_t n_dslots = 0, n_tslots = 0;
  uint32_t vsplit = 1;
  std::vector<Job> wcjobs;
  std::vector<Term> wcterms;
  std::vector<BJob> wjobs;
  std::vector<BJob> bjobs;
  std::vector<Term> bterms;
  std::vector<BTermPos> bpos;
  uint32_t b_dig_bytes = 0;
  uint32_t b_kpad_max = 0;
  uint32_t b_bits = 8;
};

static const size_t COMBINE_TREE_MIN = 12;
static const size_t BUCKET_TERMS_MAX = 589824;
class PhaseBuilder {
 public:
  PhaseBuilder(Phase& ph, uint32_t& next_partial, uint32_t fchunk, uint32_t vchunk, uint32_t bucket_min = 0, uint32_t bwin = 0,
               uint32_t vsplit = 1, uint32_t bbits = 8)
      : ph_(ph), next_partial_(next_partial), fchunk_(fchunk), vchunk_(vchunk), bucket_min_(bucket_min), bwin_(bwin),
        vsplit_(vsplit < 1 ? 1 : (vsplit > VSPLIT_MAX ? VSPLIT_MAX : vsplit)) {
    ph_.vsplit = vsplit_;
    ph_.b_bits = bbits;
  }
  void begin(uint32_t out_slot) {
    out_ = out_slot;
    f_.clear();
    v_.clear();
    a_.clear();
  }
  void fixed(uint32_t sslot, uint32_t base) { f_.push_back(Term{sslot, base}); }
  void var(uint32_t sslot, uint32_t pslot) { v_.push_back(Term{sslot, pslot}); }
  void addend(uint32_t pslot, bool negate = false) { a_.push_back(AFF_FLAG | (negate ? NEG_FLAG : 0u) | pslot); }
  void addend_j(uint32_t jslot, bool negate = false) { a_.push_back((negate ? NEG_FLAG : 0u) | jslot); }
  uint32_t new_partial() { return next_partial_++; }
  void end(bool late = false) {
    const size_t MAXP = 128;
    size_t fchunk_ = this->fchunk_, vchunk_ = this->vchunk_;
    const bool bucket = bucket_min_ && v_.size() >= bucket_min_ && v_.size() <= BUCKET_TERMS_MAX;
    if (!bucket)
      for (Term& t : v_) t = Term{dslot(t.s), tslot(t.b)};
    if ((f_.size() + fchunk_ - 1) / fchunk_ > MAXP) fchunk_ = (f_.size() + MAXP - 1) / MAXP;
    if ((v_.size() + vchunk_ - 1) / vchunk_ > MAXP) vchunk_ = (v_.size() + MAXP - 1) / MAXP;
    size_t nf = (f_.size() + fchunk_ - 1) / fchunk_, nv = bucket ? 1 : (v_.size() + vchunk_ - 1) / vchunk_;
    const bool wsplit = !bucket && vsplit_ > 1 && nv > 0;
    size_t pieces = nf + (wsplit ? 1 : nv) + a_.size();
    if (pieces == 0) throw std::logic_error("empty msm");
    bool direct = pieces == 1 && a_.empty();
    std::vector<uint32_t> parts;
    for (size_t c = 0; c < nf; ++c) {
      uint32_t out = direct ? out_ : next_partial_++;
      size_t b = c * fchunk_, e = std::min(f_.size(), b + fchunk_);
      ph_.fjobs.push_back(Job{out, (uint32_t)ph_.fterms.size(), (uint32_t)(e - b)});
      ph_.fterms.insert(ph_.fterms.end(), f_.begin() + b, f_.begin() + e);
      parts.push_back(out);
    }
    if (bucket) {
      const uint32_t out = direct ? out_ : next_partial_++;
      const uint32_t kpad = (uint32_t)((v_.size() + 63) / 64 * 64);
      BJob bj{out, next_partial_, (uint32_t)ph_.bterms.size(), (uint32_t)v_.size(), kpad, ph_.b_dig_bytes};
      next_partial_ += bwin_;
      for (size_t i = 0; i < v_.size(); ++i) ph_.bpos.push_back(BTermPos{ph_.b_dig_bytes + (uint32_t)i, kpad});
      ph_.bterms.insert(ph_.bterms.end(), v_.begin(), v_.end());
      ph_.b_dig_bytes += bwin_ * kpad;
      ph_.b_kpad_max = std::max(ph_.b_kpad_max, kpad);
      ph_.bjobs.push_back(bj);
      parts.push_back(out);
    }
    if (wsplit) {
      std::vector<uint32_t> first(nv);
      for (size_t c = 0; c < nv; ++c) {
        first[c] = next_partial_;
        next_partial_ += vsplit_;
        size_t b = c * vchunk_, e = std::min(v_.size(), b + vchunk_);
// ... 791 lines not shown
```

Before: 723,600 proofs/s.

## Use branch-free fast EC adds in MSM kernels with flagged exceptional-lane fallback

The fixed-base, remask and variable-base MSM kernels now use a fast XYZZ add/double path without the infinity and equal-point checks. Lanes whose accumulator ends degenerate are recorded in a per-stream fallback list using a wave ballot and atomics. A follow-up fix kernel recomputes only those lanes with the original checked formulas. The aim is to cut per-add branching and divergence, at the cost of an extra memset and fix-kernel launch per MSM, plus a correctness dependence on detecting every degenerate case through ZZ becoming zero.

```diff
diff --git a/include/mpshuffle.h b/include/mpshuffle.h
--- a/include/mpshuffle.h
+++ b/include/mpshuffle.h
@@ -106,6 +106,7 @@
 uint32_t mp_group_size(const mp_table* t, size_t B);
 int mp_set_group_refine(mp_table* t, uint32_t points_per_subgroup, uint32_t min_subgroups);
 uint64_t mp_reverified_count(const mp_table* t);
+uint64_t mp_fallback_lanes(mp_ctx* ctx);
 int mp_set_group_adapt(mp_table* t, int on);
 int mp_set_bucket_min(mp_table* t, size_t terms);
 int mp_set_bucket_bits(mp_table* t, uint32_t bits);
diff --git a/mental-poker_amd/_native.py b/mental-poker_amd/_native.py
--- a/mental-poker_amd/_native.py
+++ b/mental-poker_amd/_native.py
@@ -11,7 +11,7 @@
 
 SYMBOLS = [
     "mp_ctx_create", "mp_ctx_destroy", "mp_last_error", "mp_check_name", "mp_proof_size", "mp_params_size",
-    "mp_point_size", "mp_proof_size_curve", "mp_params_size_curve", "mp_set_merged_verify", "mp_set_subgroup_check", "mp_set_bucket_min", "mp_set_bucket_bits", "mp_set_bucket_split", "mp_set_validated", "mp_deck_validate_dev", "mp_set_chain_max_links", "mp_set_chain_group", "mp_set_chain_slice", "mp_chain_group_size", "mp_chain_last_slice", "mp_set_transcript_lanes", "mp_set_group_lanes", "mp_set_work_split", "mp_set_group_verify", "mp_group_size", "mp_set_group_refine", "mp_reverified_count", "mp_set_group_adapt", "mp_set_pipeline", "mp_set_plan_params", "mp_set_plan_thresholds", "mp_set_toom_cook", "mp_host_alloc", "mp_host_free", "mp_set_io_chunk", "mp_shuffle_and_remask_batch_keys", "mp_table_create_params",
+    "mp_point_size", "mp_proof_size_curve", "mp_params_size_curve", "mp_set_merged_verify", "mp_set_subgroup_check", "mp_set_bucket_min", "mp_set_bucket_bits", "mp_set_bucket_split", "mp_set_validated", "mp_deck_validate_dev", "mp_set_chain_max_links", "mp_set_chain_group", "mp_set_chain_slice", "mp_chain_group_size", "mp_chain_last_slice", "mp_set_transcript_lanes", "mp_set_group_lanes", "mp_set_work_split", "mp_set_group_verify", "mp_group_size", "mp_set_group_refine", "mp_reverified_count", "mp_fallback_lanes", "mp_set_group_adapt", "mp_set_pipeline", "mp_set_plan_params", "mp_set_plan_thresholds", "mp_set_toom_cook", "mp_host_alloc", "mp_host_free", "mp_set_io_chunk", "mp_shuffle_and_remask_batch_keys", "mp_table_create_params",
     "mp_verify_shuffle_batch_keys", "mp_shuffle_and_remask_batch_keys_dev", "mp_verify_shuffle_batch_keys_dev",
     "mp_keyset_create", "mp_keyset_destroy", "mp_keyset_size", "mp_shuffle_and_remask_batch_keyset_dev", "mp_verify_shuffle_batch_keyset_dev",
     "mp_setup", "mp_table_create", "mp_table_create_ex", "mp_table_window_bits", "mp_table_destroy", "mp_shuffle_and_remask", "mp_verify_shuffle",
@@ -134,6 +134,8 @@
     cdll.mp_reverified_count.argtypes = [c.c_void_p]
     cdll.mp_set_group_adapt.argtypes = [c.c_void_p, c.c_int]
     cdll.mp_reverified_count.restype = c.c_uint64
+    cdll.mp_fallback_lanes.argtypes = [c.c_void_p]
+    cdll.mp_fallback_lanes.restype = c.c_uint64
     cdll.mp_set_pipeline.argtypes = [c.c_void_p, c.c_int]
     cdll.mp_set_plan_params.argtypes = [c.c_void_p, c.c_int] + [c.c_uint32] * 5
     cdll.mp_set_plan_thresholds.argtypes = [c.c_void_p] + [c.c_size_t] * 5
@@ -331,6 +333,9 @@
     def check_name(self, code):
         return self.lib.mp_check_name(code).decode()
 
+    def fallback_lanes(self):
+        return int(self.lib.mp_fallback_lanes(self.h))
+
     def proof_size(self, m, n):
         return self.lib.mp_proof_size_curve(CURVE_IDS[self.curve], m, n)
 
diff --git a/mental-poker_amd/csrc/capi.hip b/mental-poker_amd/csrc/capi.hip
--- a/mental-poker_amd/csrc/capi.hip
+++ b/mental-poker_amd/csrc/capi.hip
@@ -117,6 +117,12 @@
   c->vside = rt::stream_create();
   c->h2d = c->vstream;
   c->d2h = c->vside;
+  c->fbk_streams[0] = c->stream;
+  c->fbk_streams[1] = c->vstream;
+  c->fbk_streams[2] = c->side;
+  c->fbk_streams[3] = c->vside;
+  c->fbk.alloc((size_t)4 * FBK_WORDS, c->stream);
+  rt::stream_sync(c->stream);
   c->ev_fork = rt::event_create();
   c->ev_shuf = rt::event_create();
   c->ev_tab = rt::event_create();
@@ -284,6 +290,24 @@
   std::lock_guard<std::recursive_mutex> mp_lock_(t->ctx->mu);
   t->set_group_refine(points_per_subgroup, min_subgroups);
   return MP_OK;
+}
+uint64_t mp_fallback_lanes(mp_ctx* ctx) {
+  if (!ctx) return 0;
+  std::lock_guard<std::recursive_mutex> mp_lock_(ctx->mu);
+  uint64_t sum = 0;
+  try {
+    for (rt::Stream st : ctx->fbk_streams) rt::stream_sync(st);
+    for (uint32_t r = 0; r < 4; ++r) {
+      uint64_t v = 0;
+      rt::d2h(&v, ctx->fbk.p + (size_t)r * FBK_WORDS + 2, 8, ctx->stream);
+      rt::stream_sync(ctx->stream);
+      sum += v;
+    }
+  } catch (const std::exception& e) {
+    fail(MP_ERR_INTERNAL, e.what());
+    return 0;
+  }
+  return sum;
 }
 uint64_t mp_reverified_count(const mp_table* t) {
   if (!t) return 0;
diff --git a/mental-poker_amd/csrc/curve.hpp b/mental-poker_amd/csrc/curve.hpp
--- a/mental-poker_amd/csrc/curve.hpp
+++ b/mental-poker_amd/csrc/curve.hpp
@@ -184,14 +184,8 @@
   return p;
 }
 template <class C>
-MP_HD void xyzz_dbl_ip(Xyzz<C>& p) {
-  typedef typename C::FqP F;
-  if (fe_is_zero(p.ZZ)) return;
-  if (fe_is_zero(p.Y)) {
-    p.ZZ = fe_zero<F>();
-    p.ZZZ = fe_zero<F>();
-    return;
-  }
+MP_HD void xyzz_dbl_fast(Xyzz<C>& p) {
+  typedef typename C::FqP F;
   const Fe<F> U = fe_dbl<F>(p.Y);
   const Fe<F> V = fe_sqr<F>(U);
   const Fe<F> W = fe_mul<F>(U, V);
@@ -204,17 +198,9 @@
   p.ZZ = fe_mul<F>(V, p.ZZ);
   p.ZZZ = fe_mul<F>(W, p.ZZZ);
 }
-template <class C, bool PROBE = false>
-MP_HD void xyzz_madd_signed_ip(Xyzz<C>& p, const Aff<C>& q, bool neg) {
-  typedef typename C::FqP F;
-  if (aff_is_inf<C>(q)) return;
-  if (fe_is_zero(p.ZZ)) {
-    p.X = q.x;
-    p.Y = neg ? fe_neg<F>(q.y) : q.y;
-    p.ZZ = fe_one<F>();
-    p.ZZZ = fe_one<F>();
-    return;
-  }
+template <class C>
+MP_HD Fe<typename C::FqP> aff_y_signed_lazy(const Aff<C>& q, bool neg) {
+  typedef typename C::FqP F;
   Fe<F> qy = q.y;
   if constexpr (LazySub<F>::ON) {
     const Fe<F> ny = fe_neg_lazy<F>(q.y);
@@ -223,6 +209,61 @@
   } else {
     if (neg) qy = fe_neg<F>(q.y);
   }
+  return qy;
+}
+template <class C>
+MP_HD void xyzz_madd_main(Xyzz<C>& p, const Fe<typename C::FqP>& Pd, const Fe<typename C::FqP>& Rr) {
+  typedef typename C::FqP F;
+  const Fe<F> PP = fe_sqr<F>(Pd);
+  const Fe<F> PPP = fe_mul<F>(Pd, PP);
+  const Fe<F> Q = fe_mul<F>(p.X, PP);
+  const Fe<F> X3 = fe_sub_sub_dbl<F>(fe_sqr<F>(Rr), PPP, Q);
+  p.Y = fe_mulsub<F>(Rr, fe_sub_lazy<F>(Q, X3), p.Y, PPP);
+  p.X = X3;
+  p.ZZ = fe_mul<F>(p.ZZ, PP);
+  p.ZZZ = fe_mul<F>(p.ZZZ, PPP);
+}
+template <class C>
+MP_HD void xyzz_madd_signed_fast(Xyzz<C>& p, const Aff<C>& q, bool neg) {
+  typedef typename C::FqP F;
+  const Fe<F> qy = aff_y_signed_lazy<C>(q, neg);
+  const Fe<F> Pd = fe_sub_wide<F>(fe_mul<F>(q.x, p.ZZ), p.X);
+  const Fe<F> Rr = fe_sub_wide<F>(fe_mul<F>(qy, p.ZZZ), p.Y);
+  xyzz_madd_main<C>(p, Pd, Rr);
+}
+template <class C>
+MP_HD void xyzz_madd_fast(Xyzz<C>& p, const Aff<C>& q) {
+  xyzz_madd_signed_fast<C>(p, q, false);
+}
+template <class C>
+MP_HD void xyzz_set_signed(Xyzz<C>& p, const Aff<C>& q, bool neg) {
+  typedef typename C::FqP F;
+  p.X = q.x;
+  p.Y = neg ? fe_neg<F>(q.y) : q.y;
+  p.ZZ = fe_one<F>();
+  p.ZZZ = fe_one<F>();
+}
+
+template <class C>
+MP_HD void xyzz_dbl_ip(Xyzz<C>& p) {
+  typedef typename C::FqP F;
+  if (fe_is_zero(p.ZZ)) return;
+  if (fe_is_zero(p.Y)) {
+    p.ZZ = fe_zero<F>();
+    p.ZZZ = fe_zero<F>();
+    return;
+  }
+  xyzz_dbl_fast<C>(p);
+}
+template <class C, bool PROBE = false>
+MP_HD void xyzz_madd_signed_ip(Xyzz<C>& p, const Aff<C>& q, bool neg) {
+  typedef typename C::FqP F;
+  if (aff_is_inf<C>(q)) return;
+  if (fe_is_zero(p.ZZ)) {
+    xyzz_set_signed<C>(p, q, neg);
+    return;
+  }
+  const Fe<F> qy = aff_y_signed_lazy<C>(q, neg);
   const Fe<F> Pd = fe_sub_wide<F>(fe_mul<F>(q.x, p.ZZ), p.X);
   const Fe<F> Rr = fe_sub_wide<F>(fe_mul<F>(qy, p.ZZZ), p.Y);
   if (fe_is_zero(Pd)) {
@@ -234,14 +275,7 @@
     }
     return;
   }
-  const Fe<F> PP = fe_sqr<F>(Pd);
-  const Fe<F> PPP = fe_mul<F>(Pd, PP);
-  const Fe<F> Q = fe_mul<F>(p.X, PP);
-  const Fe<F> X3 = fe_sub_sub_dbl<F>(fe_sqr<F>(Rr), PPP, Q);
-  p.Y = fe_mulsub<F>(Rr, fe_sub_lazy<F>(Q, X3), p.Y, PPP);
-  p.X = X3;
-  p.ZZ = fe_mul<F>(p.ZZ, PP);
-  p.ZZZ = fe_mul<F>(p.ZZZ, PPP);
+  xyzz_madd_main<C>(p, Pd, Rr);
 }
 template <class C, bool PROBE = false>
 MP_HD void xyzz_madd_ip(Xyzz<C>& p, const Aff<C>& q) {
diff --git a/mental-poker_amd/csrc/engine_base.hpp b/mental-poker_amd/csrc/engine_base.hpp
--- a/mental-poker_amd/csrc/engine_base.hpp
+++ b/mental-poker_amd/csrc/engine_base.hpp
@@ -116,6 +116,8 @@
   uint32_t sq_exp[12] = {0};
   mp::Profiler prof;
   uint32_t bk_slots = 0;
+  mp::DevBuf<uint32_t> fbk;
+  mp::rt::Stream fbk_streams[4]{};
 };
 namespace mp {
 struct LaneSwap {
@@ -149,6 +151,21 @@
     ctx->prof.begin(#NAME, ctx->stream, (uint64_t)(nx) * (ny)); \
     MP_LAUNCH(NAME, C, ctx->stream, (nx), (ny), (args));   \
     ctx->prof.end(ctx->stream);                            \
+  } while (0)
+inline uint32_t* mp_fallback_list(mp_ctx* c) {
+  for (uint32_t r = 0; r < 4; ++r)
+    if (c->fbk_streams[r] == c->stream) return c->fbk.p + (size_t)r * mp::FBK_WORDS;
+  throw std::runtime_error("fast MSM kernel launched on a stream that has no fallback list");
+}
+#define MP_RUN_FAST(NAME, FIX, C, nx, ny, args)                                   \
+  do {                                                                            \
+    if ((nx) > 0 && (ny) > 0) {                                                   \
+      (args).fl = mp_fallback_list(ctx);                                          \
+      mp::rt::dzero((args).fl, 4, ctx->stream);                                   \
+      MP_RUN(NAME, C, (nx), (ny), (args));                                        \
+      const mp::FixArgs<decltype(args)> fx_{(args), (uint32_t)(nx), (uint32_t)(ny)}; \
+      MP_RUN(FIX, C, mp::FIX_THREADS, 1, fx_);                                    \
+    }                                                                             \
   } while (0)
 
 struct mp_io_stage {
diff --git a/mental-poker_amd/csrc/engine_core.hpp b/mental-poker_amd/csrc/engine_core.hpp
--- a/mental-poker_amd/csrc/engine_core.hpp
+++ b/mental-poker_amd/csrc/engine_core.hpp
@@ -703,22 +703,26 @@
         FixedQuadArgs qa{a, B, ph.n_f};
         MP_WAVE_RUN(k_fixed_msm_q, C, quad_waves(B, ph.n_f), 0, qa);
       } else {
-        MP_RUN(k_fixed_msm, C, B, ph.n_f, a);
+        MP_RUN_FAST(k_fixed_msm, k_fixed_fix, C, B, ph.n_f, a);
       }
     }
     if (ph.n_v) {
       VarArgs a{w.D.p, w.T.p, w.J.p, ph.vjobs.p, ph.vterms.p, w.Bpad, nwin, ph.vsplit};
       const uint32_t nvl = ph.n_v * ph.vsplit;
 #ifdef MP_EXP_VAR_LDS
+      a.fl = mp_fallback_list(ctx);
+      rt::dzero(a.fl, 4, ctx->stream);
       ctx->prof.begin("k_var_msm", ctx->stream);
       hipLaunchKernelGGL((k_var_msm<C>), dim3((B + 255u) / 256u, nvl), dim3(256), MP_EXP_VAR_LDS, ctx->stream, a, (uint32_t)B);
       ctx->prof.end(ctx->stream);
+      const FixArgs<VarArgs> fx{a, B, nvl};
+      MP_RUN(k_var_fix, C, FIX_THREADS, 1, fx);
 #else
       if (quad_ops(B, nvl)) {
         VarQuadArgs qa{a, B, nvl};
         MP_WAVE_RUN(k_var_msm_q, C, quad_waves(B, nvl), 0, qa);
       } else {
-        MP_RUN(k_var_msm, C, B, nvl, a);
+        MP_RUN_FAST(k_var_msm, k_var_fix, C, B, nvl, a);
       }
 #endif
       if (ph.n_wc) {
@@ -935,13 +939,13 @@
         rt::event_record(ctx->ev_fork, s);
         ctx->stream = ctx->side;
         rt::stream_wait(ctx->side, ctx->ev_fork);
-        MP_RUN(k_remask, C, B, 2 * N, ra);
+        MP_RUN_FAST(k_remask, k_remask_fix, C, B, 2 * N, ra);
         run_phase(pph[0], w, B, PH_NORM, l.shuf);
         rt::event_record(ctx->ev_shuf, ctx->side);
         prove_side_work(q, w, B, true);
         rt::event_record(ctx->ev_tab, ctx->side);
       } else {
-        MP_RUN(k_remask, C, B, 2 * N, ra);
+        MP_RUN_FAST(k_remask, k_remask_fix, C, B, 2 * N, ra);
       }
       if (overlap) {
         prove_init(ia, B);
@@ -1521,7 +1525,7 @@
     MP_RUN(k_chain_tile, C, Tq * chain.K, 1, ta);
     run_bucket(w, ph, chain_cs.p, Tpad, chain_d8.p, (size_t)ph.b_dig_bytes, Tq, Tq, "chain verification: too many tables for one launch", gt.p, chain.K);
     FixedArgs fx{chain_cs.p, w.J.p, FB.p, ph.fjobs.p, ph.fterms.p, w.Bpad, fbg, Tpad};
-    MP_RUN(k_fixed_msm, C, Tq, ph.n_f, fx);
+    MP_RUN_FAST(k_fixed_msm, k_fixed_fix, C, Tq, ph.n_f, fx);
     if (ph.n_c0) {
       CombineArgs cb0{w.J.p, w.P.p, ph.cjobs0.p, ph.cterms0.p, w.Bpad};
       MP_RUN(k_combine, C, Tq, ph.n_c0, cb0);
@@ -1713,7 +1717,7 @@
     }
     run_bucket(w, ph, chain_cs.p, Tpad, chain_d8.p, (size_t)ph.b_dig_bytes, T, T, "group verification: too many groups for one launch", tile, gplan.K);
     FixedArgs fx{chain_cs.p, w.J.p, FB.p, ph.fjobs.p, ph.fterms.p, w.Bpad, fbg, Tpad};
-    MP_RUN(k_fixed_msm, C, T, ph.n_f, fx);
+    MP_RUN_FAST(k_fixed_msm, k_fixed_fix, C, T, ph.n_f, fx);
     if (ph.n_c0) {
       CombineArgs cb0{w.J.p, w.P.p, ph.cjobs0.p, ph.cterms0.p, w.Bpad};
       MP_RUN(k_combine, C, T, ph.n_c0, cb0);
@@ -1754,7 +1758,7 @@
     LoadScalarsArgs sa{drho.p, w.S.p, w.status.p, w.Bpad, 1, 0};
     MP_RUN(k_load_scalars, C, B, 1, sa);
     RemaskArgs ra{w.S.p, w.P.p, w.J.p, FB.p, nullptr, w.Bpad, 1, 0, 0, 2, fb.G(), fb.pk(), fbg, 0, nullptr, nullptr, 0, 0, 0};
-    MP_RUN(k_remask, C, B, 2, ra);
+    MP_RUN_FAST(k_remask, k_remask_fix, C, B, 2, ra);
     normalize_flat(w.J.p + j_off<C>(2, w.Bpad, 0), w.P.p + p_off<C>(2, w.Bpad, 0), w.NS.p, (size_t)2 * w.Bpad);
     StorePointsArgs st{dout.p, w.P.p, w.Bpad, 2, 2};
     MP_RUN(k_store_points, C, B, 2, st);
diff --git a/mental-poker_amd/csrc/kernels_msm.hpp b/mental-poker_amd/csrc/kernels_msm.hpp
--- a/mental-poker_amd/csrc/kernels_msm.hpp
+++ b/mental-poker_amd/csrc/kernels_msm.hpp
@@ -71,6 +71,20 @@
   return a;
 }
 template <class C>
+MP_HD Aff<C> ld_aff_chk(const uint32_t* p, bool& inf) {
+  typedef typename C::FqP F;
+  uint32_t w[Geo<C>::PW];
+  ld_words<Geo<C>::PW>(p, w);
+  uint32_t o = 0;
+#pragma unroll
+  for (uint32_t i = 0; i < Geo<C>::PW; ++i) o |= w[i];
+  inf = o == 0;
+  Aff<C> a;
+  a.x = fe_unpack<F>(w);
+  a.y = fe_unpack<F>(w + Geo<C>::FW);
+  return a;
+}
+template <class C>
 MP_HD void st_aff(uint32_t* p, const Aff<C>& a) {
   st_fe<typename C::FqP>(p, a.x);
   st_fe<typename C::FqP>(p + Geo<C>::FW, a.y);
@@ -97,6 +111,83 @@
 MP_HD size_t p_off(uint32_t slot, uint32_t Bpad, uint32_t b) { return ((size_t)slot * Bpad + b) * Geo<C>::PW; }
 template <class C>
 MP_HD size_t j_off(uint32_t slot, uint32_t Bpad, uint32_t b) { return ((size_t)slot * Bpad + b) * Geo<C>::JW; }
+
+static const uint32_t FIX_THREADS = 64u * 2048u;
+
+template <class C, bool FAST>
+struct Chain {
+  Xyzz<C> acc = xyzz_inf<C>();
+  bool started = false;
+  MP_HD void add(const uint32_t* p, bool neg) {
+    if constexpr (FAST) {
+      bool inf;
+      const Aff<C> q = ld_aff_chk<C>(p, inf);
+      if (inf) return;
+      if (started) {
+        xyzz_madd_signed_fast<C>(acc, q, neg);
+      } else {
+        xyzz_set_signed<C>(acc, q, neg);
+        started = true;
+      }
+    } else {
+      xyzz_madd_signed_ip<C>(acc, ld_aff<C>(p), neg);
+    }
+  }
+  MP_HD void dbl() {
+    if constexpr (FAST)
+      xyzz_dbl_fast<C>(acc);
+    else
+      xyzz_dbl_ip<C>(acc);
+  }
+  MP_HD bool bad() const { return FAST && started && fe_is_zero(acc.ZZ); }
+};
+MP_HD void fallback_flag(uint32_t* fl, uint32_t b, uint32_t y, bool bad) {
+#if defined(__HIP_DEVICE_COMPILE__)
+  const unsigned long long m = __ballot(bad);
+  if (m == 0) return;
+  if ((b & 63u) == (uint32_t)(__ffsll(m) - 1)) {
+    const uint32_t e = atomicAdd(fl, 1u);
+    if (e < FBK_CAP)
+      *reinterpret_cast<uint4*>(fl + FBK_HDR + 4 * e) = make_uint4(b & ~63u, y, (uint32_t)m, (uint32_t)(m >> 32));
+    atomicAdd(reinterpret_cast<unsigned long long*>(fl + 2), (unsigned long long)__popcll(m));
+  }
+#else
+  if (!bad) return;
+  const uint32_t e = __atomic_fetch_add(fl, 1u, __ATOMIC_RELAXED);
+  const unsigned long long m = 1ull << (b & 63u);
+  if (e < FBK_CAP) {
+    uint32_t* en = fl + FBK_HDR + 4 * e;
+    en[0] = b & ~63u;
+    en[1] = y;
+    en[2] = (uint32_t)m;
+    en[3] = (uint32_t)(m >> 32);
+  }
+  __atomic_fetch_add(reinterpret_cast<unsigned long long*>(fl + 2), 1ull, __ATOMIC_RELAXED);
+#endif
+}
+template <class A>
+struct FixArgs {
+  A a;
+  uint32_t nx, ny;
+};
+template <class A, class Body>
+MP_HD void fallback_run(const FixArgs<A>& f, uint32_t x, Body&& body) {
+  const uint32_t* fl = f.a.fl;
+  const uint32_t n = fl[0], lane = x & 63u, wave = x >> 6, nwaves = FIX_THREADS >> 6;
+  if (n <= FBK_CAP) {
+    for (uint32_t e = wave; e < n; e += nwaves) {
+      const uint32_t* en = fl + FBK_HDR + 4 * e;
+      const unsigned long long m = (unsigned long long)en[2] | (unsigned long long)en[3] << 32;
+      if ((m >> lane) & 1ull) body(en[0] + lane, en[1]);
+    }
+  } else {
+    const uint32_t wx = (f.nx + 63u) / 64u;
+    for (size_t e = wave; e < (size_t)wx * f.ny; e += nwaves) {
+      const uint32_t b = (uint32_t)(e % wx) * 64u + lane, y = (uint32_t)(e / wx);
+      if (b < f.nx) body(b, y);
+    }
+  }
+}
 
 struct FbGeom {
   uint32_t bits, windows, entries;
@@ -110,6 +201,7 @@
   uint32_t Bpad;
   FbGeom g;
   uint32_t Sbpad;
+  uint32_t* fl;
 };
 template <class C>
 MP_HD const uint32_t* fb_entry(const uint32_t* FB, const FbGeom& g, uint32_t base, uint32_t w, uint32_t d) {
@@ -121,11 +213,11 @@
   if (off + g.bits > 32 && word < 7) v |= k[word + 1] << (32 - off);
   return v & ((1u << g.bits) - 1u);
 }
-template <class C>
-MP_HD void body_fixed_msm(const FixedArgs& a, uint32_t b, uint32_t y) {
+template <class C, bool FAST>
+MP_HD void body_fixed_msm_t(const FixedArgs& a, uint32_t b, uint32_t y) {
   typedef typename C::FrP R;
   const Job job = a.jobs[y];
-  Xyzz<C> acc = xyzz_inf<C>();
+  Chain<C, FAST> ch;
   for (uint32_t t = 0; t < job.count; ++t) {
     const Term term = a.terms[job.begin + t];
     uint32_t k[8];
@@ -133,12 +225,22 @@
 #pragma unroll 1
     for (uint32_t w = 0; w < a.g.windows; ++w) {
       const uint32_t d = fb_digit(k, a.g, w);
-      if (d) xyzz_madd_ip<C>(acc, ld_aff<C>(fb_entry<C>(a.FB, a.g, term.b, w, d)));
-    }
-  }
-  st_jac<C>(a.J + j_off<C>(job.out, a.Bpad, b), xyzz_to_jac<C>(acc));
+      if (d) ch.add(fb_entry<C>(a.FB, a.g, term.b, w, d), false);
+    }
+  }
+  st_jac<C>(a.J + j_off<C>(job.out, a.Bpad, b), xyzz_to_jac<C>(ch.acc));
+  if constexpr (FAST) fallback_flag(a.fl, b, y, ch.bad());
+}
+template <class C>
+MP_HD void body_fixed_msm(const FixedArgs& a, uint32_t b, uint32_t y) {
+  body_fixed_msm_t<C, true>(a, b, y);
 }
 MP_KERNEL_OCC(k_fixed_msm, FixedArgs, body_fixed_msm, Geo<C>::OCC4)
+template <class C>
+MP_HD void body_fixed_fix(const FixArgs<FixedArgs>& f, uint32_t x, uint32_t) {
+  fallback_run(f, x, [&](uint32_t b, uint32_t y) { body_fixed_msm_t<C, false>(f.a, b, y); });
+}
+MP_KERNEL_OCC(k_fixed_fix, FixArgs<FixedArgs>, body_fixed_fix, Geo<C>::OCC4)
 
 struct RemaskArgs {
   const uint32_t* S;
@@ -158,9 +260,10 @@
   const uint32_t* kidx;
   FbGeom kg;
   uint32_t nkeys;
-};
-template <class C>
-MP_HD void body_remask(const RemaskArgs& a, uint32_t b, uint32_t y) {
+  uint32_t* fl;
+};
+template <class C, bool FAST>
+MP_HD void body_remask_t(const RemaskArgs& a, uint32_t b, uint32_t y) {
   typedef typename C::FrP R;
   const uint32_t i = y >> 1, comp = y & 1;
   uint32_t src = a.perm ? a.perm[(size_t)b * a.N + i] : i;
@@ -168,42 +271,45 @@
   uint32_t k[8];
   fe_to_canonical<R>(ld_fe<R>(a.S + s_off(a.s_rho + i, a.Bpad, b)), k);
   const uint32_t base = comp ? a.base_pk : a.base_G;
-  Xyzz<C> acc = xyzz_inf<C>();
+  Chain<C, FAST> ch;
   if (a.keyed == 2 && comp) {
     uint32_t key = a.kidx[b];
     if (key >= a.nkeys) key = 0;
 #pragma unroll 1
     for (uint32_t w = 0; w < a.kg.windows; ++w) {
       const uint32_t d = fb_digit(k, a.kg, w);
-      if (d) xyzz_madd_ip<C>(acc, ld_aff<C>(fb_entry<C>(a.KFB, a.kg, key, w, d)));
-    }
-    xyzz_madd_ip<C>(acc, ld_aff<C>(a.P + p_off<C>(a.p_deck + 2 * src + comp, a.Bpad, b)));
-    st_jac<C>(a.J + j_off<C>(a.j_out + y, a.Bpad, b), xyzz_to_jac<C>(acc));
-    return;
-  }
-  if (a.keyed && comp) {
+      if (d) ch.add(fb_entry<C>(a.KFB, a.kg, key, w, d), false);
+    }
+  } else if (a.keyed && comp) {
 #pragma unroll 1
     for (uint32_t w = 0; w < a.nwin; ++w) {
       const int d = a.D[((size_t)(a.d_first + i) * a.nwin + w) * a.Bpad + b];
       if (d != 0) {
         const uint32_t e = (uint32_t)(d < 0 ? -d : d) - 1;
-        const Aff<C> q = ld_aff<C>(a.T + p_off<C>((a.t_first + w) * VB_ENTRIES + e, a.Bpad, b));
-        xyzz_madd_signed_ip<C>(acc, q, d < 0);
+        ch.add(a.T + p_off<C>((a.t_first + w) * VB_ENTRIES + e, a.Bpad, b), d < 0);
       }
     }
-    xyzz_madd_ip<C>(acc, ld_aff<C>(a.P + p_off<C>(a.p_deck + 2 * src + comp, a.Bpad, b)));
-    st_jac<C>(a.J + j_off<C>(a.j_out + y, a.Bpad, b), xyzz_to_jac<C>(acc));
-    return;
-  }
-#pragma unroll 1
-  for (uint32_t w = 0; w < a.g.windows; ++w) {
-    const uint32_t d = fb_digit(k, a.g, w);
-    if (d) xyzz_madd_ip<C>(acc, ld_aff<C>(fb_entry<C>(a.FB, a.g, base, w, d)));
-  }
-  xyzz_madd_ip<C>(acc, ld_aff<C>(a.P + p_off<C>(a.p_deck + 2 * src + comp, a.Bpad, b)));
-  st_jac<C>(a.J + j_off<C>(a.j_out + y, a.Bpad, b), xyzz_to_jac<C>(acc));
+  } else {
+#pragma unroll 1
+    for (uint32_t w = 0; w < a.g.windows; ++w) {
+      const uint32_t d = fb_digit(k, a.g, w);
+      if (d) ch.add(fb_entry<C>(a.FB, a.g, base, w, d), false);
+    }
+  }
+  ch.add(a.P + p_off<C>(a.p_deck + 2 * src + comp, a.Bpad, b), false);
+  st_jac<C>(a.J + j_off<C>(a.j_out + y, a.Bpad, b), xyzz_to_jac<C>(ch.acc));
+  if constexpr (FAST) fallback_flag(a.fl, b, y, ch.bad());
+}
+template <class C>
+MP_HD void body_remask(const RemaskArgs& a, uint32_t b, uint32_t y) {
+  body_remask_t<C, true>(a, b, y);
 }
 MP_KERNEL_OCC(k_remask, RemaskArgs, body_remask, Geo<C>::OCC4)
+template <class C>
+MP_HD void body_remask_fix(const FixArgs<RemaskArgs>& f, uint32_t x, uint32_t) {
+  fallback_run(f, x, [&](uint32_t b, uint32_t y) { body_remask_t<C, false>(f.a, b, y); });
+}
+MP_KERNEL_OCC(k_remask_fix, FixArgs<RemaskArgs>, body_remask_fix, Geo<C>::OCC4)
 
 struct KeyTermsArgs {
   const uint32_t* S;
@@ -442,19 +548,20 @@
   const Term* terms;
   uint32_t Bpad, nwin;
   uint32_t split;
-};
-template <class C>
-MP_HD void body_var_msm(const VarArgs& a, uint32_t b, uint32_t y) {
+  uint32_t* fl;
+};
+template <class C, bool FAST>
+MP_HD void body_var_msm_t(const VarArgs& a, uint32_t b, uint32_t y) {
   const uint32_t jidx = a.split > 1 ? y / a.split : y, r = y - jidx * a.split;
   const Job job = a.jobs[jidx];
   const int w_top = a.split > 1 ? (int)vsplit_lo(r + 1, a.split, a.nwin) - 1 : (int)a.nwin - 1;
   const int w_low = a.split > 1 ? (int)vsplit_lo(r, a.split, a.nwin) : 0;
-  Xyzz<C> acc = xyzz_inf<C>();
+  Chain<C, FAST> ch;
 #pragma unroll 1
   for (int w = w_top; w >= w_low; --w) {
     if (w != w_top) {
 #pragma unroll 1
-      for (int q = 0; q < VB_WINDOW_BITS; ++q) xyzz_dbl_ip<C>(acc);
+      for (int q = 0; q < VB_WINDOW_BITS; ++q) ch.dbl();
     }
 #pragma unroll 1
     for (uint32_t t = 0; t < job.count; ++t) {
@@ -462,14 +569,23 @@
       const int d = a.D[((size_t)term.s * a.nwin + w) * a.Bpad + b];
       if (d != 0) {
         const uint32_t e = (uint32_t)(d < 0 ? -d : d) - 1;
-        const Aff<C> q = ld_aff<C>(a.T + p_off<C>(term.b * VB_ENTRIES + e, a.Bpad, b));
-        xyzz_madd_signed_ip<C>(acc, q, d < 0);
+        ch.add(a.T + p_off<C>(term.b * VB_ENTRIES + e, a.Bpad, b), d < 0);
       }
     }
   }
-  st_jac<C>(a.J + j_off<C>(job.out + r, a.Bpad, b), xyzz_to_jac<C>(acc));
+  st_jac<C>(a.J + j_off<C>(job.out + r, a.Bpad, b), xyzz_to_jac<C>(ch.acc));
+  if constexpr (FAST) fallback_flag(a.fl, b, y, ch.bad());
+}
+template <class C>
+MP_HD void body_var_msm(const VarArgs& a, uint32_t b, uint32_t y) {
+  body_var_msm_t<C, true>(a, b, y);
 }
 MP_KERNEL_OCC(k_var_msm, VarArgs, body_var_msm, Geo<C>::OCC_VAR)
+template <class C>
+MP_HD void body_var_fix(const FixArgs<VarArgs>& f, uint32_t x, uint32_t) {
+  fallback_run(f, x, [&](uint32_t b, uint32_t y) { body_var_msm_t<C, false>(f.a, b, y); });
+}
+MP_KERNEL_OCC(k_var_fix, FixArgs<VarArgs>, body_var_fix, Geo<C>::OCC_VAR)
 
 struct CombineArgs {
   uint32_t* J;
@@ -710,13 +826,16 @@
 
 #define MP_MSM_KERNELS(X, C) \
   MP_KERNEL_INST(X, k_fixed_msm, FixedArgs, C) \
+  MP_KERNEL_INST(X, k_fixed_fix, FixArgs<FixedArgs>, C) \
   MP_KERNEL_INST(X, k_remask, RemaskArgs, C) \
+  MP_KERNEL_INST(X, k_remask_fix, FixArgs<RemaskArgs>, C) \
   MP_KERNEL_INST(X, k_key_windows, KeyWinArgs, C) \
   MP_KERNEL_INST(X, k_key_terms, KeyTermsArgs, C) \
   MP_KERNEL_INST(X, k_gather_keys, GatherKeysArgs, C) \
   MP_KERNEL_INST(X, k_recode, RecodeArgs, C) \
   MP_KERNEL_INST(X, k_table, TableArgs, C) \
   MP_KERNEL_INST(X, k_var_msm, VarArgs, C) \
+  MP_KERNEL_INST(X, k_var_fix, FixArgs<VarArgs>, C) \
   MP_KERNEL_INST(X, k_combine, CombineArgs, C) \
   MP_KERNEL_INST(X, k_normalize, NormArgs, C) \
   MP_KERNEL_INST(X, k_normalize_multi, NormMultiArgs, C) \
diff --git a/mental-poker_amd/csrc/layout.hpp b/mental-poker_amd/csrc/layout.hpp
--- a/mental-poker_amd/csrc/layout.hpp
+++ b/mental-poker_amd/csrc/layout.hpp
@@ -52,6 +52,9 @@
 static inline int vb_windows(int scalar_bits) { return (scalar_bits + 1 + VB_WINDOW_BITS - 1) / VB_WINDOW_BITS; }
 MP_HD uint32_t vsplit_lo(uint32_t r, uint32_t k, uint32_t nwin) { return r * nwin / k; }
 static const uint32_t VSPLIT_MAX = 16;
+static const uint32_t FBK_CAP = 8192;
+static const uint32_t FBK_HDR = 8;
+static const uint32_t FBK_WORDS = FBK_HDR + 4 * FBK_CAP;
 
 struct Phase {
   std::vector<Term> recode;
```

Result: no change. 729,600 proofs/s, median of 6 (+0.8%).
